# anneouyang/OuterSPACE

Measured on AMD Instinct MI355X. Metric: spgemm_output_nnz_per_s, higher is better.
Workload: dtype f64

## Files before the change

### outerspace_amd/csrc/osp_pipeline.h

```cpp
#pragma once

#define OSP_WITH_RA(ctx_, ...)                                               \
    do {                                                                     \
        if ((ctx_)->rank_atomic) { constexpr bool RA = true; __VA_ARGS__; }  \
        else { constexpr bool RA = false; __VA_ARGS__; }                     \
    } while (0)

template <class T> struct Producer {
    virtual ~Producer() {}
    virtual void produce(uint64_t r0, uint64_t r1, bool whole, uint64_t base, uint64_t count,
                         Part<T> *stage, PhaseTimer &tm, const uint32_t *cells = nullptr, Part<T> *qstage = nullptr,
                         const HubArgs *hub = nullptr, bool compact = false, bool has_long = true, bool desc_only = false, bool walk_all = false) = 0;
};

template <class T> struct MergeIO {
    Part<T> *stage;
    const uint64_t *row_off; uint64_t r0, r1, base;
    int64_t *c_rowptr; uint32_t *c_col; T *c_val;
    const uint64_t *out_in; uint64_t *out_out;
    ChunkTable<T> ct{};
    uint32_t *abort_word = nullptr;
    const RunDesc<T> *runs0 = nullptr; const uint32_t *rowfirst0 = nullptr; const uint32_t *b_colidx = nullptr; const T *b_vals = nullptr;
};
template <class T> struct ShortRuns {
    const RunDesc<T> *runs0 = nullptr; const uint32_t *rowfirst0 = nullptr; const uint32_t *b_colidx = nullptr; const T *b_vals = nullptr;
};

struct TilePlan {
    uint32_t *tile_rows = nullptr;
    uint32_t ntiles = 0;
    uint32_t *long_rows = nullptr;
    uint32_t nlong = 0;
};

static TilePlan plan_tiles(Context *ctx, Scratch &sc, const uint64_t *row_off, uint64_t r0, uint64_t r1, uint64_t base,
                           uint32_t cap, uint32_t max_rows, const uint8_t *force_start, uint64_t total, uint64_t nforce) {
    hipStream_t s = ctx->stream;
    const uint64_t nr = r1 - r0;
    TilePlan pl;
    uint32_t *flag_scan = sc.get<uint32_t>(nr + 1);
    uint32_t *tmp_rows = sc.get<uint32_t>(nr + 1);
    uint64_t *scan_tmp = sc.get<uint64_t>(scan_scratch_entries(std::max<uint64_t>(nr + 1, 16)));
    const uint64_t slot = 8ull * cap;
    CoarseStartFlag csf{row_off, r0, base, slot, force_start};
    device_exclusive_scan<CoarseStartFlag, uint32_t>(csf, nr, flag_scan, (uint32_t *)scan_tmp, s);
    compact_flagged_kernel<CoarseStartFlag><<<grid_for(nr, 256), 256, 0, s>>>(csf, flag_scan, nr, r0, tmp_rows);
    const uint32_t ncb = (uint32_t)std::min<uint64_t>(nr, 2 + nforce + total / slot + nr / 65536);
    const uint32_t *ncb_p = flag_scan + nr;
    uint32_t *cb_cnt = sc.get<uint32_t>((uint64_t)ncb + 1);
    tile_walk_kernel<<<grid_for(ncb, 128), 128, 0, s>>>(tmp_rows, ncb_p, ncb, r1, row_off, cap, max_rows, nullptr, cb_cnt, nullptr);
    device_exclusive_scan<LoadU32, uint32_t>(LoadU32{cb_cnt}, ncb, cb_cnt, (uint32_t *)scan_tmp, s);
    HeavyRowFlag hrf{row_off, r0, cap};
    uint32_t *long_scan = sc.get<uint32_t>(nr + 1);
    uint32_t *long_tmp = sc.get<uint32_t>(scan_scratch_entries(std::max<uint64_t>(nr + 1, 16)));
    device_exclusive_scan<HeavyRowFlag, uint32_t>(hrf, nr, long_scan, long_tmp, s);
    pl.long_rows = sc.get<uint32_t>(nr + 1);
    compact_flagged_kernel<HeavyRowFlag><<<grid_for(nr, 256), 256, 0, s>>>(hrf, long_scan, nr, r0, pl.long_rows);
    { Gather g(s); g.add(&pl.ntiles, (const uint32_t *)cb_cnt + ncb); g.add(&pl.nlong, (const uint32_t *)long_scan + nr); g.wait(); }
    pl.tile_rows = sc.get<uint32_t>((uint64_t)pl.ntiles + 1);
    tile_walk_kernel<<<grid_for(ncb, 128), 128, 0, s>>>(tmp_rows, ncb_p, ncb, r1, row_off, cap, max_rows, cb_cnt, nullptr, pl.tile_rows);
    return pl;
}

struct DirectSrc {
    const uint32_t *rowfirst; const uint64_t *off; const uint32_t *bs; const uint32_t *perm; const uint32_t *b_colidx;
    uint64_t *chunk_off;
    uint64_t direct_max;
    const int64_t *b_rowptr = nullptr;
    uint64_t K = 0, nnz_b = 0;
    Scratch *keep = nullptr;
    mutable HubTables hub{};
    mutable bool hub_refused = false;
    bool gather = false;
    bool expand_rows = false;
    mutable bool chunk_off_ready = true;
    const uint32_t *rows_sorted = nullptr;
    const uint64_t *row_off = nullptr;
    uint64_t rw_cap = 0, nnz = 0;
    void ensure_chunk_off(hipStream_t s) const {
        if (chunk_off_ready) return;
        sym_scatter_offsets_kernel<<<grid_for(nnz, 256), 256, 0, s>>>(perm, off, rows_sorted, row_off, rw_cap, nnz, chunk_off);
        chunk_off_ready = true;
    }
    const void *a_vals = nullptr, *b_vals = nullptr;
    bool av_in_order = false;
    unsigned long long *gstat = nullptr;
};

template <class T> struct PanelPlan {
    Scratch sc;
    TilePlan p0;
    uint32_t max_rows = 0;
    uint64_t *hoff = nullptr, *hscan_tmp = nullptr, *blkbase = nullptr, *hbase = nullptr, *vbase = nullptr, *cellbase = nullptr;
    uint8_t *hbits = nullptr, *hmode = nullptr;
    uint32_t *nstretch = nullptr;
    uint64_t nh = 0, nblocks = 0, nvirt = 0, ncell = 0;
    uint64_t mode_rows[3] = {0, 0, 0}, mode_partials[3] = {0, 0, 0};
    uint32_t *ghist = nullptr, *ghist_tmp = nullptr;
    Part<T> *qstage = nullptr;
    uint64_t *vrow_off = nullptr;
    uint8_t *vfirst = nullptr;
    uint32_t *vcol0 = nullptr, *vcol1 = nullptr;
    uint32_t *cells = nullptr;
    HubArgs hub{};
    GatherArgs<T> ga{};
    uint32_t *vrun_off = nullptr, *vrun_end = nullptr;
    uint32_t *nwritten = nullptr;
    uint64_t *xjobbase = nullptr;
    uint64_t xjobs_bound = 0, xpartials = 0;
    bool expand_ok = false;
    bool may_write = false;
    const DirectSrc *split_from_b = nullptr;
    bool split_beside = false;
    explicit PanelPlan(Context *c) : sc(c) {}
};

__global__ void mode_totals_kernel(const uint32_t *rows, uint32_t nlong, const uint64_t *row_off, const uint8_t *hmode,
                                   const uint8_t *hsmall, unsigned long long *totals) {
    uint64_t part[3] = {0, 0, 0}, cnt[3] = {0, 0, 0}, nsmall = 0;
    for (uint32_t h = blockIdx.x * blockDim.x + threadIdx.x; h < nlong; h += gridDim.x * blockDim.x) {
        const uint64_t U = row_off[rows[h] + 1] - row_off[rows[h]];
        const uint8_t m = hmode[h];
        nsmall += hsmall[h] ? 1ull : 0ull;
#pragma unroll
        for (int mode = 0; mode < 3; mode++) { part[mode] += m == mode ? U : 0ull; cnt[mode] += m == mode ? 1ull : 0ull; }
    }
    for (uint8_t mode = 0; mode < 3; mode++) {
        const uint64_t p = wave_reduce_sum<uint64_t>(part[mode]), c = wave_reduce_sum<uint64_t>(cnt[mode]);
        if (lane_id() == 0 && c) { atomicAdd(&totals[mode], (unsigned long long)c); atomicAdd(&totals[3 + mode], (unsigned long long)p); }
    }
    nsmall = wave_reduce_sum<uint64_t>(nsmall);
    if (lane_id() == 0 && nsmall) atomicAdd(&totals[6], (unsigned long long)nsmall);
}

template <class T>
static void plan_panel(Context *ctx, Result *res, PhaseTimer &tm, PanelPlan<T> &pl, const uint64_t *row_off, uint64_t r0, uint64_t r1,
                       uint64_t base, uint64_t count, int colbits, const DirectSrc *ds) {
    hipStream_t s = ctx->stream;
    Scratch &sc = pl.sc;
    constexpr uint32_t kCap = (uint32_t)TileCap<T>::value;
    pl.max_rows = (uint32_t)std::min<uint64_t>(kTileMaxRows, colbits >= 32 ? 1ull : (1ull << (32 - colbits)));
    pl.p0 = plan_tiles(ctx, sc, row_off, r0, r1, base, kCap, pl.max_rows, nullptr, count, 0);
    res->info.light_tiles += pl.p0.ntiles - pl.p0.nlong;
    if (!pl.p0.nlong) return;
    const uint32_t nlong = pl.p0.nlong;
    pl.hoff = sc.get<uint64_t>((uint64_t)nlong + 1);
    pl.hscan_tmp = sc.get<uint64_t>(scan_scratch_entries(nlong));
    device_exclusive_scan<HeavyLen, uint64_t>(HeavyLen{pl.p0.long_rows, row_off}, nlong, pl.hoff, pl.hscan_tmp, s);
    pl.hbits = sc.get<uint8_t>(nlong);
    pl.hmode = sc.get<uint8_t>(nlong);
    pl.nstretch = sc.get<uint32_t>(nlong);
    uint32_t *nseg = sc.get<uint32_t>(nlong);
    uint64_t *nhist = sc.get<uint64_t>(nlong), *ncellh = sc.get<uint64_t>(nlong);
    const bool want_gather = ds && ds->gather;
    uint64_t *nrund = want_gather ? sc.get<uint64_t>(nlong) : nullptr, *rdbase = want_gather ? sc.get<uint64_t>((uint64_t)nlong + 1) : nullptr;
    uint64_t nrd = 0;
    pl.blkbase = sc.get<uint64_t>((uint64_t)nlong + 1); pl.hbase = sc.get<uint64_t>((uint64_t)nlong + 1);
    pl.vbase = sc.get<uint64_t>((uint64_t)nlong + 1); pl.cellbase = sc.get<uint64_t>((uint64_t)nlong + 1);
    unsigned long long *totals = (unsigned long long *)sc.get<uint64_t>(7);
    uint8_t *hsmall = sc.get<uint8_t>(nlong);
    SmallLimits small_lim{};
    if (want_gather && !(getenv("OSP_PLAN_SMALL") && atoi(getenv("OSP_PLAN_SMALL")) == 0) &&
        !(getenv("OSP_GATHER_OVER") && atoi(getenv("OSP_GATHER_OVER")) == 0)) {
        small_lim.cells = (uint32_t)std::clamp<long>(getenv("OSP_PLAN_SMALL_CELLS") ? atol(getenv("OSP_PLAN_SMALL_CELLS")) : (long)kSmallCells,
                                                     (long)kSmallCellsMin, (long)kSmallCellsMax);
        small_lim.chunks = (uint32_t)std::clamp<long>(getenv("OSP_PLAN_SMALL_CHUNKS") ? atol(getenv("OSP_PLAN_SMALL_CHUNKS")) : (long)kSmallChunks,
                                                      1L, (long)kSmallChunks);
    }
    uint64_t nsmall = 0;
    const uint64_t row_max = getenv("OSP_SPLIT_ROW_MAX") ? strtoull(getenv("OSP_SPLIT_ROW_MAX"), nullptr, 10) : kSplitRowMax;
    const int bits_cap = std::max(colbits - kDenseBits, 1);
    const int hub_b_want = std::min(kSplitMaxBits, bits_cap);
    const bool hub_env = !(getenv("OSP_HUB") && atoi(getenv("OSP_HUB")) == 0);
    int hub_b = 0;
    uint64_t ndcell = 0, tot[6] = {0, 0, 0, 0, 0, 0};
    const int direct_fine = 2;
    const double hub_min_share = getenv("OSP_HUB_MIN_SHARE") ? atof(getenv("OSP_HUB_MIN_SHARE")) : 0.2;
    bool hub_decided = false;
    for (int attempt = 0; attempt < 3; attempt++) {
        const bool hub_possible = ds && ds->b_rowptr && ds->keep && ctx->rank_atomic && hub_env && !ds->hub_refused;
        if (!hub_possible) hub_b = 0;
        split_params_kernel<<<grid_for(nlong, 256), 256, 0, s>>>(pl.p0.long_rows, nlong, row_off, colbits, row_max, bits_cap, ds ? ds->rowfirst : nullptr,
                                                                 ds ? ds->direct_max : 0ull, kCap, pl.hbits, pl.hmode, pl.nstretch, nseg, nhist, ncellh,
                                                                 hub_b, direct_fine, ds ? nrund : nullptr, hsmall, ds ? small_lim : SmallLimits{});
        zero_async(s, {{totals, 7 * sizeof(uint64_t)}});
        mode_totals_kernel<<<std::min(grid_for(nlong, 256), 64u), 256, 0, s>>>(pl.p0.long_rows, nlong, row_off, pl.hmode, hsmall, totals);
        device_exclusive_scan<LoadU32As64, uint64_t>(LoadU32As64{pl.nstretch}, nlong, pl.blkbase, pl.hscan_tmp, s);
        device_exclusive_scan<LoadU32As64, uint64_t>(LoadU32As64{nseg}, nlong, pl.vbase, pl.hscan_tmp, s);
        device_exclusive_scan<LoadU64, uint64_t>(LoadU64{nhist}, nlong, pl.hbase, pl.hscan_tmp, s);
        if (ds) device_exclusive_scan<LoadU64, uint64_t>(LoadU64{ncellh}, nlong, pl.cellbase, pl.hscan_tmp, s);
        if (ds && nrund) device_exclusive_scan<LoadU64, uint64_t>(LoadU64{nrund}, nlong, rdbase, pl.hscan_tmp, s);
        ndcell = 0;
        nrd = 0;
        {
            Gather g(s);
            g.add(&pl.nh, (const uint64_t *)pl.hoff + nlong); g.add(&pl.nblocks, (const uint64_t *)pl.blkbase + nlong);
            g.add(&pl.nvirt, (const uint64_t *)pl.vbase + nlong); g.add(&pl.ncell, (const uint64_t *)pl.hbase + nlong);
            if (ds) g.add(&ndcell, (const uint64_t *)pl.cellbase + nlong);
            if (ds && nrund) g.add(&nrd, (const uint64_t *)rdbase + nlong);
            for (int i = 0; i < 6; i++) g.add(&tot[i], (const uint64_t *)totals + i);
            g.add(&nsmall, (const uint64_t *)totals + 6);
            g.wait();
        }
        if (ds && ndcell >= 0xffffffffull) { ds = nullptr; hub_b = 0; continue; }
        if (hub_possible && !hub_decided && hub_b == 0 && pl.nblocks && (double)tot[3 + kModeStretch] >= hub_min_share * (double)count) {
            hub_decided = true;
            hub_b = hub_b_want;
            continue;
        }
        break;
    }
    for (int m = 0; m < 3; m++) { pl.mode_rows[m] = tot[m]; pl.mode_partials[m] = tot[3 + m]; }
    if (pl.nh >= 0xffffffffull) throw Error(OSP_ERR_CAPACITY, "long rows of one panel exceed 2^32 partial products");
    res->info.heavy_rows += nlong;
    res->info.heavy_partials += pl.nh;
    res->info.direct_rows += pl.mode_rows[kModeDirect];
    res->info.direct_partials += pl.mode_partials[kModeDirect];
    if (pl.ncell >= 0xffffffffull || pl.nblocks >= 0x7fffffffull || pl.nvirt >= 0xffffffffull || ndcell >= 0xffffffffull)
        throw Error(OSP_ERR_CAPACITY, "split histogram too large");
    if (getenv("OSP_VERBOSE"))
        fprintf(stderr, "[osp]   panel rows [%llu,%llu): %u tiles, %u long rows with %llu partial products -> %llu segments; direct: %llu rows, %llu "
                        "partial products, %llu cells\n",
                (unsigned long long)r0, (unsigned long long)r1, pl.p0.ntiles, nlong, (unsigned long long)pl.nh, (unsigned long long)pl.nvirt,
                (unsigned long long)pl.mode_rows[kModeDirect], (unsigned long long)pl.mode_partials[kModeDirect], (unsigned long long)ndcell);
    pl.ghist = sc.get<uint32_t>(pl.ncell + 1);
    pl.ghist_tmp = sc.get<uint32_t>(scan_scratch_entries(pl.ncell + 1));
    pl.vrow_off = sc.get<uint64_t>(pl.nvirt + 1);
    pl.vfirst = sc.get<uint8_t>(pl.nvirt + 1);
    pl.vcol0 = sc.get<uint32_t>(pl.nvirt + 1);
    pl.vcol1 = sc.get<uint32_t>(pl.nvirt + 1);
    if (pl.mode_rows[kModeDirect]) {
        pl.cells = sc.get<uint32_t>(ndcell);
        GatherPlan gp{};
        RunDesc<T> *runs = nullptr;
        static const uint64_t max_runs = getenv("OSP_GATHER_MAX_RUNS") ? strtoull(getenv("OSP_GATHER_MAX_RUNS"), nullptr, 10) : 0xffffffffull;
        if (ds->gather && nrund && nrd < max_runs) {
            runs = sc.get<RunDesc<T>>(std::max<uint64_t>(nrd, 1));
            pl.vrun_off = sc.get<uint32_t>(pl.nvirt + 1);
            pl.vrun_end = sc.get<uint32_t>(pl.nvirt + 1);
            gp.rdbase = rdbase; gp.vrun_off = pl.vrun_off; gp.vrun_end = pl.vrun_end;
            gp.rowruns = sc.get<uint32_t>(nlong);
            pl.nwritten = gp.nwritten = sc.get<uint32_t>(1);
            fill_async(s, {{pl.vrun_off, (pl.nvirt + 1) * sizeof(uint32_t), kNoRuns}, {gp.rowruns, (uint64_t)nlong * sizeof(uint32_t), kNoRuns},
                           {pl.nwritten, sizeof(uint32_t), 0u}});
            gp.over = !(getenv("OSP_GATHER_OVER") && atoi(getenv("OSP_GATHER_OVER")) == 0);
            gp.av_in_order = ds->av_in_order ? 1u : 0u;
            pl.may_write = !gp.over;
            pl.ga.runs = runs; pl.ga.b_colidx = ds->b_colidx; pl.ga.b_vals = (const T *)ds->b_vals;
        }
        if (!(runs && gp.over) || (hub_b && pl.nblocks)) ds->ensure_chunk_off(s);
        gp.mark_skipped = ds->chunk_off_ready ? 1u : 0u;
        const bool plan_small = runs != nullptr && gp.over && nsmall != 0;
        const bool plan_big = !plan_small || nsmall < pl.mode_rows[kModeDirect];
        if (plan_small) gp.small = hsmall;
        if (getenv("OSP_VERBOSE"))
            fprintf(stderr, "[osp]   small planner: %llu of %llu direct rows (at most %u chunks, %u cells)\n", (unsigned long long)(plan_small ? nsmall : 0),
                    (unsigned long long)pl.mode_rows[kModeDirect], small_lim.chunks, small_lim.cells);
        tm.begin(PH_PLAN_K, s);
        if (plan_small)
            direct_plan_small_kernel<T><<<nlong, kWave, direct_plan_small_lds(small_lim.cells), s>>>(
                pl.p0.long_rows, nlong, pl.hbits, nseg, pl.vbase, pl.hoff, colbits, kCap, ds->rowfirst, ds->off, ds->bs, ds->perm, ds->b_colidx,
                pl.vrow_off, pl.vcol0, pl.vcol1, ds->chunk_off, gp, (const T *)ds->a_vals, runs);
        if (!plan_big) {  }
        else if (nlong <= 4u * ctx->cus)
            direct_plan_kernel<T, kDirectCellsBig><<<nlong, kDirectThreads, 0, s>>>(pl.p0.long_rows, nlong, pl.hmode, pl.hbits, nseg, pl.vbase, pl.hoff,
                                                                                 pl.cellbase, row_off, colbits, kCap, ds->rowfirst, ds->off, ds->bs, ds->perm,
                                                                                 ds->b_colidx, pl.vrow_off, pl.vcol0, pl.vcol1, pl.cells, ds->chunk_off, gp,
                                                                                 (const T *)ds->a_vals, runs);
        else
        direct_plan_kernel<T><<<nlong, kDirectThreads, 0, s>>>(pl.p0.long_rows, nlong, pl.hmode, pl.hbits, nseg, pl.vbase, pl.hoff, pl.cellbase, row_off,
                                                              colbits, kCap, ds->rowfirst, ds->off, ds->bs, ds->perm, ds->b_colidx, pl.vrow_off,
                                                              pl.vcol0, pl.vcol1, pl.cells, ds->chunk_off, gp, (const T *)ds->a_vals, runs);
        tm.end(PH_PLAN_K);
        if (gp.rowruns && ds->gstat) gather_stats_kernel<<<std::min(grid_for(nlong, 256), 64u), 256, 0, s>>>(pl.p0.long_rows, nlong, row_off, gp.rowruns, ds->gstat);
#ifdef OSP_PLAN_PROF
        if (getenv("OSP_VERBOSE")) {
            unsigned long long hp[8] = {0}, z[8] = {0};
            OSP_HIP(hipStreamSynchronize(s));
            (void)hipMemcpyFromSymbol(hp, HIP_SYMBOL(osp_plan_prof), sizeof(hp));
            (void)hipMemcpyToSymbol(HIP_SYMBOL(osp_plan_prof), z, sizeof(z));
            double tot = 0;
            for (int k = 0; k < 6; k++) tot += (double)hp[k];
            fprintf(stderr, "[osp]   planner cycles: header %.1f %%, chunk descriptors %.1f %%, histogram pass %.1f %%, grouping %.1f %%, cell pass %.1f %%, "
                            "prefixes + output %.1f %%; %.0f cycles per row, %u rows\n", 100 * hp[0] / tot, 100 * hp[1] / tot, 100 * hp[2] / tot, 100 * hp[3] / tot,
                    100 * hp[4] / tot, 100 * hp[5] / tot, tot / std::max(1u, nlong), nlong);
            (void)hipMemcpyFromSymbol(hp, HIP_SYMBOL(osp_plan_small_prof), sizeof(hp));
            (void)hipMemcpyToSymbol(HIP_SYMBOL(osp_plan_small_prof), z, sizeof(z));
            tot = 0;
            for (int k = 0; k < 5; k++) tot += (double)hp[k];
            if (plan_small && tot > 0)
                fprintf(stderr, "[osp]   small planner cycles: header + chunk descriptors %.1f %%, histogram pass %.1f %%, grouping %.1f %%, counts %.1f %%, "
                                "prefixes + output %.1f %%; %.0f cycles per row, %llu rows\n", 100 * hp[0] / tot, 100 * hp[1] / tot, 100 * hp[2] / tot,
                        100 * hp[3] / tot, 100 * hp[4] / tot, tot / (double)nsmall, (unsigned long long)nsmall);
        }
#endif
        res->info.direct_plan_launches++;
        dbg_sync(s, "plan of the direct rows");
    }
    if (hub_b && pl.nblocks) {
        if (!ds->hub.sx) {
            Scratch &keep = *ds->keep;
            const uint64_t nb = ds->nnz_b;
            Scratch tmp(ctx);
            uint8_t *rowstart = tmp.get<uint8_t>(nb + 4);
            uint32_t *sx = keep.get<uint32_t>(nb + 1), *runstart = keep.get<uint32_t>(nb + 1);
            uint16_t *runblk = keep.get<uint16_t>(nb + 2);
            uint32_t *scan_tmp = tmp.get<uint32_t>(scan_scratch_entries(nb + 1));
            OSP_HIP(hipMemsetAsync(rowstart, 0, nb + 4, s));
            hub_rowstart_kernel<<<grid_for(ds->K, 256), 256, 0, s>>>(ds->b_rowptr, ds->K, rowstart);
            const int sh = colbits - hub_b;
            const HubRunFlag flag{rowstart, ds->b_colidx, sh};
            device_exclusive_scan<HubRunFlag, uint32_t>(flag, nb, sx, scan_tmp, s);
            compact_flagged_kernel<HubRunFlag><<<grid_for(nb, 256), 256, 0, s>>>(flag, sx, nb, 0, runstart);
            hub_runstart_end_kernel<<<1, 1, 0, s>>>(sx + nb, runstart, (uint32_t)nb);
            OSP_HIP(hipMemsetAsync(runblk, 0, (nb + 2) * sizeof(uint16_t), s));
            hub_runblk_kernel<<<std::min(grid_for(nb, 256), 4096u), 256, 0, s>>>(sx + nb, runstart, ds->b_colidx, sh, runblk);
            OSP_HIP(hipStreamSynchronize(s));
            ds->hub.sx = sx; ds->hub.runstart = runstart; ds->hub.runblk = runblk; ds->hub.sh = sh;
        }
        tm.begin(PH_HUB_K, s);
        uint64_t *jobruns = sc.get<uint64_t>(pl.nblocks + 1);
        uint64_t *jobscan_tmp = sc.get<uint64_t>(scan_scratch_entries(pl.nblocks + 1));
        const size_t hub_lds = sizeof(uint32_t) << hub_b;
        hub_plan_kernel<false><<<(unsigned)pl.nblocks, kHubThreads, hub_lds, s>>>(pl.p0.long_rows, nlong, pl.blkbase, pl.hbase, pl.hbits, pl.nstretch, row_off,
                                                                           ds->rowfirst, ds->off, ds->bs, ds->perm, ds->b_colidx, ds->hub, pl.ghist,
                                                                           pl.hoff, jobruns, nullptr, nullptr, nullptr);
        device_exclusive_scan<LoadU32, uint32_t>(LoadU32{pl.ghist}, pl.ncell, pl.ghist, pl.ghist_tmp, s);
        device_exclusive_scan<LoadU64, uint64_t>(LoadU64{jobruns}, pl.nblocks, jobruns, jobscan_tmp, s);
        const uint64_t ncells = d2h(jobruns + pl.nblocks, s);
        if (ncells >= (1ull << 40)) throw Error(OSP_ERR_CAPACITY, "hub rows: too many runs in one panel");
        if (getenv("OSP_VERBOSE"))
            fprintf(stderr, "[osp]   hub rows: %llu rows, %llu products in %llu runs (%.2f records per run), %llu jobs, 2^%d blocks\n",
                    (unsigned long long)pl.mode_rows[kModeStretch], (unsigned long long)pl.mode_partials[kModeStretch], (unsigned long long)ncells,
                    ncells ? (double)pl.mode_partials[kModeStretch] / (double)ncells : 0.0, (unsigned long long)pl.nblocks, hub_b);
        const double min_run = getenv("OSP_HUB_MIN_RUN") ? atof(getenv("OSP_HUB_MIN_RUN")) : 4.0;
        const double run = ncells ? (double)pl.mode_partials[kModeStretch] / (double)ncells : 0.0;
        const bool accept = run >= min_run;
        if (!accept) {
            ds->hub_refused = true;
            tm.end(PH_HUB_K);
        } else {
            uint32_t *hcells = sc.get<uint32_t>(ncells);
            ds->ensure_chunk_off(s);
            hub_plan_kernel<true><<<(unsigned)pl.nblocks, kHubThreads, hub_lds, s>>>(pl.p0.long_rows, nlong, pl.blkbase, pl.hbase, pl.hbits, pl.nstretch, row_off,
                                                                              ds->rowfirst, ds->off, ds->bs, ds->perm, ds->b_colidx, ds->hub, pl.ghist,
                                                                              pl.hoff, nullptr, jobruns, hcells, ds->chunk_off);
            tm.end(PH_HUB_K);
            pl.hub.cells = hcells;
            pl.hub.sx = ds->hub.sx;
            res->info.hub_plan_launches++;
            res->info.hub_cells += ncells;
            res->info.hub_rows += pl.mode_rows[kModeStretch];
            res->info.hub_partials += pl.mode_partials[kModeStretch];
        }
        dbg_sync(s, "plan of the hub rows");
    }
    if (ds && ds->expand_rows) {
        pl.expand_ok = true;
        const bool hubs = pl.hub.cells != nullptr;
        const int from_b_env = getenv("OSP_SPLIT_FROM_B") ? atoi(getenv("OSP_SPLIT_FROM_B")) : 1;
        if (!hubs && pl.nblocks != 0 && from_b_env != 0) pl.split_from_b = ds;
        pl.split_beside = from_b_env != 2;
        const bool stretch_x = !hubs && !pl.split_from_b;
        const uint64_t rows_x = pl.mode_rows[kModeSplitRow] + (stretch_x ? pl.mode_rows[kModeStretch] : 0);
        pl.xpartials = pl.mode_partials[kModeSplitRow] + (stretch_x ? pl.mode_partials[kModeStretch] : 0);
        if (getenv("OSP_VERBOSE") && pl.nblocks && !hubs)
            fprintf(stderr, "[osp]   stretch rows: %llu rows, %llu partial products split %s\n", (unsigned long long)pl.mode_rows[kModeStretch],
                    (unsigned long long)pl.mode_partials[kModeStretch], pl.split_from_b ? (pl.split_beside ? "from B" : "from B, after the join") : "from staged records");
        if (rows_x) {
            pl.xjobbase = sc.get<uint64_t>((uint64_t)nlong + 1);
            device_exclusive_scan<ExpandJobs, uint64_t>(ExpandJobs{pl.p0.long_rows, row_off, pl.hmode, kModeSplitRow, stretch_x ? kModeStretch : kModeSplitRow},
                                                        nlong, pl.xjobbase, pl.hscan_tmp, s);
            pl.xjobs_bound = pl.xpartials / kExpandJob + rows_x;
        }
    }
}

template <class T>
static void split_stretch_from_b(Context *ctx, hipStream_t s, const PanelPlan<T> &pl, const uint64_t *row_off, uint64_t base, int colbits) {
    const DirectSrc *ds = pl.split_from_b;
    const TilePlan &p0 = pl.p0;
    const uint32_t nlong = p0.nlong;
    const uint32_t *perm = ds->av_in_order ? nullptr : ds->perm;
    const RowSrc<float> cols{ds->rowfirst, ds->off, ds->bs, nullptr, nullptr, ds->b_colidx, nullptr};
    const RowSrc<T> src{ds->rowfirst, ds->off, ds->bs, perm, (const T *)ds->a_vals, ds->b_colidx, (const T *)ds->b_vals};
    split_count_kernel<true><<<(unsigned)pl.nblocks, kSplitThreads, 0, s>>>(p0.long_rows, nlong, pl.blkbase, pl.hbase, pl.hbits, pl.nstretch, row_off, base, colbits,
                                                                          nullptr, 0u, pl.ghist, cols);
    device_exclusive_scan<LoadU32, uint32_t>(LoadU32{pl.ghist}, pl.ncell, pl.ghist, pl.ghist_tmp, s);
    OSP_WITH_RA(ctx, split_scatter_kernel<T, RA, true><<<(unsigned)pl.nblocks, kSplitThreads, 0, s>>>(
                         p0.long_rows, nlong, pl.blkbase, pl.hbase, pl.hbits, pl.nstretch, row_off, base, colbits, nullptr, pl.ghist, pl.hoff, pl.qstage, src));
    split_vrows_kernel<<<grid_for(pl.nvirt + 1, 256), 256, 0, s>>>(nlong, pl.vbase, pl.hbase, pl.nstretch, pl.hbits, pl.hmode, colbits, pl.ghist, pl.hoff, pl.nvirt,
                                                                  pl.nh, pl.vrow_off, pl.vfirst, pl.vcol0, pl.vcol1);
    OSP_HIP(hipGetLastError());
}

template <class T>
static void merge_panel(Context *ctx, Result *res, PhaseTimer &tm, const MergeIO<T> &io, int colbits, PanelPlan<T> &pl) {
    hipStream_t s = ctx->stream;
    Scratch &sc = pl.sc;
    constexpr uint32_t kCap = (uint32_t)TileCap<T>::value;
    const uint32_t max_rows = pl.max_rows;
#ifdef OSP_CHECK_DESC
    crumbs_init();
#endif
    const uint64_t r1 = io.r1, base = io.base;
    const TilePlan &p0 = pl.p0;

    MergeLevels<T> lv{};
    lv.stage[0] = io.stage; lv.row_off[0] = io.row_off; lv.base[0] = base; lv.c_rowptr[0] = io.c_rowptr; lv.heavy_nnz[0] = nullptr;
    uint32_t ntot = p0.ntiles;
    TileDesc *desc = nullptr;
    TilePlan p1;
    uint64_t *vbase = pl.vbase;
    int64_t *vptr = nullptr;
    uint64_t *seg_src = nullptr;
    uint32_t *seg_nnz = nullptr;
    Part<T> *qstage = pl.qstage;
    if (p0.nlong) {
        const uint32_t nlong = p0.nlong;
        uint64_t *hoff = pl.hoff, *hscan_tmp = pl.hscan_tmp, *blkbase = pl.blkbase, *hbase = pl.hbase;
        uint8_t *hbits = pl.hbits;
        uint32_t *nstretch = pl.nstretch, *ghist = pl.ghist, *ghist_tmp = pl.ghist_tmp;
        const uint64_t nh = pl.nh, nblocks = pl.nblocks, nvirt = pl.nvirt, ncell = pl.ncell;
        uint64_t *vrow_off = pl.vrow_off;
        uint8_t *vfirst = pl.vfirst;
        if (pl.mode_rows[kModeSplitRow]) {
            tm.begin(PH_SPLIT_K);
            OSP_WITH_RA(ctx, split_row_kernel<T, RA><<<nlong, kSplitRowThreads, 0, s>>>(p0.long_rows, nlong, hbits, pl.hmode, vbase, hoff, io.row_off,
                                                                                     base, colbits, io.stage, qstage, vrow_off));
            tm.end(PH_SPLIT_K);
            res->info.split_launches++;
            res->info.split_partials += pl.mode_partials[kModeSplitRow];
            dbg_sync(s, "split: one-workgroup rows");
        }
        if (pl.split_from_b && !pl.split_beside) split_stretch_from_b<T>(ctx, s, pl, io.row_off, base, colbits);
        if (nblocks && !pl.hub.cells && !pl.split_from_b) {
            split_count_kernel<<<(unsigned)nblocks, kSplitThreads, 0, s>>>(p0.long_rows, nlong, blkbase, hbase, hbits, nstretch, io.row_off,
                                                                         base, colbits, (const char *)io.stage, (uint32_t)sizeof(Part<T>), ghist);
            device_exclusive_scan<LoadU32, uint32_t>(LoadU32{ghist}, ncell, ghist, ghist_tmp, s);
            OSP_WITH_RA(ctx, split_scatter_kernel<T, RA><<<(unsigned)nblocks, kSplitThreads, 0, s>>>(
                                 p0.long_rows, nlong, blkbase, hbase, hbits, nstretch, io.row_off, base, colbits, io.stage, ghist, hoff, qstage));
        }
        dbg_sync(s, "split: stretch rows");
        if (!pl.split_from_b)
            split_vrows_kernel<<<grid_for(nvirt + 1, 256), 256, 0, s>>>(nlong, vbase, hbase, nstretch, hbits, pl.hmode, colbits, ghist, hoff, nvirt, nh,
                                                                       vrow_off, vfirst, pl.vcol0, pl.vcol1);
        OSP_HIP(hipGetLastError());
        dbg_sync(s, "split: segment offsets");
        p1 = plan_tiles(ctx, sc, vrow_off, 0, nvirt, 0, kCap, max_rows, vfirst, nh, nlong);
        dbg_sync(s, "tiles over the segments");
        vptr = (int64_t *)sc.get<uint64_t>(nvirt + 1);
        lv.stage[1] = qstage; lv.row_off[1] = vrow_off; lv.base[1] = 0; lv.c_rowptr[1] = vptr;
        if (p1.nlong) {
            const uint32_t nseg_long = p1.nlong;
            seg_src = sc.get<uint64_t>(nseg_long);
            seg_nnz = sc.get<uint32_t>(nvirt + 1);
            lv.heavy_nnz[1] = seg_nnz;
            if (pl.ga.runs) {
                uint64_t *xsjob = sc.get<uint64_t>((uint64_t)nseg_long + 1);
                uint64_t *xsjob_tmp = sc.get<uint64_t>(scan_scratch_entries((uint64_t)nseg_long + 1));
                device_exclusive_scan<SegExpandJobs, uint64_t>(SegExpandJobs{p1.long_rows, vrow_off, pl.vrun_off}, nseg_long, xsjob, xsjob_tmp, s);
                const uint64_t job_bound = nh / kExpandJob + nseg_long;
                expand_segments_kernel<T><<<(unsigned)std::min<uint64_t>(job_bound, (uint64_t)ctx->cus * 8), kExpandThreads, 0, s>>>(
                    p1.long_rows, nseg_long, xsjob, vrow_off, pl.vrun_off, pl.vrun_end, pl.ga.runs, pl.ga.b_colidx, pl.ga.b_vals, qstage);
            }
            const uint32_t *rest_list = p1.long_rows;
            uint32_t nrest = nseg_long;
            uint32_t *hscan = sc.get<uint32_t>((uint64_t)nseg_long + 1);
            uint64_t *sscan_tmp = sc.get<uint64_t>(scan_scratch_entries(nseg_long));
            {
                const SegDenseFlag df{p1.long_rows, pl.vcol0, pl.vcol1, getenv("OSP_DENSE_SEG") ? atoi(getenv("OSP_DENSE_SEG")) : 1};
                device_exclusive_scan<SegDenseFlag, uint32_t>(df, nseg_long, hscan, (uint32_t *)sscan_tmp, s);
                const uint32_t ndense = d2h(hscan + nseg_long, s);
                if (ndense) {
                    uint32_t *dense_list = sc.get<uint32_t>(ndense), *others = sc.get<uint32_t>(nseg_long - ndense);
                    seg_split_list_kernel<SegDenseFlag><<<grid_for(nseg_long, 256), 256, 0, s>>>(df, hscan, nseg_long, dense_list, others);
                    if (ctx->dense_atomic[sizeof(T) == 8])
                        dense_segment_kernel<T, true><<<grid_for(ndense, kDenseWaves), kDenseWaves * kWave, 0, s>>>(dense_list, ndense, vrow_off, pl.vcol0, pl.vcol1,
                                                                              qstage, seg_nnz);
                    else
                        dense_segment_kernel<T, false><<<grid_for(ndense, kDenseWaves), kDenseWaves * kWave, 0, s>>>(dense_list, ndense, vrow_off, pl.vcol0, pl.vcol1,
                                                                              qstage, seg_nnz);
                    res->info.dense_segments += ndense;
                    rest_list = others;
                    nrest = nseg_long - ndense;
                }
            }
            dbg_sync(s, "over-long segments: dense accumulation");
            const uint32_t big_cap = getenv("OSP_BIGTILE_CAP") ? std::min<uint32_t>((uint32_t)strtoul(getenv("OSP_BIGTILE_CAP"), nullptr, 10), kBigTileCap)
                                                                : (uint32_t)kBigTileCap;
            uint32_t nhuge = 0, nmid = 0;
            uint32_t *huge_list = nullptr, *mid_list = nullptr;
            if (nrest) {
                const SegHugeFlag hf{rest_list, vrow_off, big_cap};
                device_exclusive_scan<SegHugeFlag, uint32_t>(hf, nrest, hscan, (uint32_t *)sscan_tmp, s);
                nhuge = d2h(hscan + nrest, s);
                nmid = nrest - nhuge;
                huge_list = sc.get<uint32_t>(nhuge);
                mid_list = sc.get<uint32_t>(nmid);
                seg_partition_kernel<<<grid_for(nrest, 256), 256, 0, s>>>(hf, hscan, nrest, huge_list, mid_list);
            }
            res->info.sorted_segments += nhuge;
            if (nmid) {
                TileDesc *bdesc = sc.get<TileDesc>(nmid);
                seg_tile_desc_kernel<<<grid_for(nmid, 256), 256, 0, s>>>(mid_list, nmid, vrow_off, pl.vcol0, pl.vcol1, bdesc);
                uint32_t *bticket = sc.get<uint32_t>(1);
                zero_async(s, {{bticket, sizeof(uint32_t)}});
                const uint32_t bgrid = ctx->cus * (uint32_t)merge_wgs_per_cu<T, kBigTileThreads, kBigTileCap>();
                OSP_WITH_RA(ctx, merge_tiles_kernel<T, kBigTileThreads, 32, kBigTileCap, kMergeMaxWgs, RA>
                            <<<std::min<uint32_t>(nmid, bgrid), kBigTileThreads, 0, s>>>(bdesc, nmid, lv, colbits, nullptr, bticket, nullptr, nullptr,
                                                                                         nullptr, nullptr));
            }
            dbg_sync(s, "over-long segments: big in-place tiles");
            if (nhuge) {
                uint64_t *soff = sc.get<uint64_t>((uint64_t)nhuge + 1);
                device_exclusive_scan<HeavyLen, uint64_t>(HeavyLen{huge_list, vrow_off}, nhuge, soff, sscan_tmp, s);
                const uint64_t ns = d2h(soff + nhuge, s);
                res->info.sorted_partials += ns;
                SortedRuns runs(sc, ns);
                heavy_fill_kernel<<<grid_for(ns, 256), 256, 0, s>>>(huge_list, soff, nhuge, vrow_off, 0, colbits, (const char *)qstage,
                                                                    (uint32_t)sizeof(Part<T>), ns, runs.keys[0], runs.poss[0]);
                runs.sort(colbits + bits_for(nhuge));
                T *sorted_val = sc.get<T>(ns);
                heavy_gather_kernel<T><<<grid_for(ns, 256), 256, 0, s>>>(runs.poss[runs.cur], qstage, ns, sorted_val);
                runs.heads();
                heavy_reduce_kernel<T><<<grid_for(ns, 256), 256, 0, s>>>(runs.keys[runs.cur], sorted_val, runs.headscan, runs.head_pos(), ns, huge_list,
                                                                         soff, nhuge, vrow_off, 0, colbits, qstage);
                heavy_rows_kernel<<<grid_for(nhuge, 256), 256, 0, s>>>(huge_list, soff, nhuge, runs.headscan, seg_nnz);
            }
            dbg_sync(s, "over-long segments: global sort");
            heavy_src_inplace_kernel<<<grid_for(nseg_long, 256), 256, 0, s>>>(p1.long_rows, nseg_long, vrow_off, 0, seg_src);
        }
        lv.heavy_nnz[1] = seg_nnz;
        uint32_t *j0 = sc.get<uint32_t>(nlong), *tb = sc.get<uint32_t>((uint64_t)nlong + 1), *extra = sc.get<uint32_t>((uint64_t)nlong + 1);
        chain_rows_kernel<<<grid_for(nlong + 1, 256), 256, 0, s>>>(p0.long_rows, nlong, p0.tile_rows, p0.ntiles, vbase, p1.tile_rows,
                                                                  p1.ntiles, j0, tb, extra);
        device_exclusive_scan<LoadU32, uint32_t>(LoadU32{extra}, nlong, extra, (uint32_t *)hscan_tmp, s);
        ntot = p0.ntiles + (p1.ntiles - nlong);
        desc = sc.get<TileDesc>(ntot);
        tile_desc_kernel<(int)kCap><<<grid_for(p0.ntiles, 256), 256, 0, s>>>(p0.tile_rows, p0.ntiles, r1, io.row_off, base, 0u, j0, extra,
                                                                           nlong, tb, pl.vcol0, pl.vcol1, desc, nullptr, nullptr, io.rowfirst0);
        tile_desc_kernel<(int)kCap><<<grid_for(p1.ntiles, 256), 256, 0, s>>>(p1.tile_rows, p1.ntiles, nvirt, vrow_off, 0, 1u, j0, extra,
                                                                           nlong, tb, pl.vcol0, pl.vcol1, desc, pl.ga.runs ? pl.vrun_off : nullptr,
                                                                           pl.vrun_end);
        dbg_sync(s, "tile chain");
    } else {
        desc = sc.get<TileDesc>(ntot);
        tile_desc_kernel<(int)kCap><<<grid_for(p0.ntiles, 256), 256, 0, s>>>(p0.tile_rows, p0.ntiles, r1, io.row_off, base, 0u, nullptr,
                                                                           nullptr, 0u, nullptr, nullptr, nullptr, desc, nullptr, nullptr, io.rowfirst0);
    }
    uint64_t *tile_status = sc.get<uint64_t>(ntot);
    const uint32_t nshards = 1u;
    uint32_t *ticket = sc.get<uint32_t>((uint64_t)(nshards + 1) * kTicketStride);
    zero_async(s, {{tile_status, (uint64_t)ntot * sizeof(uint64_t)}, {ticket, (uint64_t)(nshards + 1) * kTicketStride * sizeof(uint32_t)}});
    dbg_sync(s, "tile planning, splits, over-long segments");
    tm.begin(PH_MERGE_K);
    if (io.ct.enabled) {
        const uint32_t rw_grid = ctx->cus * (uint32_t)merge_wgs_per_cu<T, kMergeThreads, TileCap<T>::value, kMergeMaxWgs, 64>();
        OSP_WITH_RA(ctx, merge_tiles_kernel<T, kMergeThreads, 64, TileCap<T>::value, kMergeMaxWgs, RA>
                    <<<std::min<uint32_t>(ntot, rw_grid), kMergeThreads, 0, s>>>(desc, ntot, lv, colbits, tile_status, ticket, io.out_in, io.c_col,
                                                                                 io.c_val, io.out_out, io.ct, nshards, io.abort_word));
    } else if (pl.ga.runs || io.runs0) {
        GatherArgs<T> ga = pl.ga;
        ga.runs0 = io.runs0;
        if (io.runs0) { ga.b_colidx = io.b_colidx; ga.b_vals = io.b_vals; }
        const uint32_t merge_grid = ctx->cus * (uint32_t)merge_wgs_per_cu<T, kMergeThreads, TileCap<T>::value>();
        OSP_WITH_RA(ctx, merge_tiles_kernel<T, kMergeThreads, 0, TileCap<T>::value, kMergeMaxWgs, RA, true>
                    <<<std::min<uint32_t>(ntot, merge_grid), kMergeThreads, 0, s>>>(desc, ntot, lv, colbits, tile_status, ticket, io.out_in, io.c_col,
                                                                                    io.c_val, io.out_out, ChunkTable<T>{}, nshards, io.abort_word, ga));
    } else {
        const uint32_t merge_grid = ctx->cus * (uint32_t)merge_wgs_per_cu<T, kMergeThreads, TileCap<T>::value>();
        OSP_WITH_RA(ctx, merge_tiles_kernel<T, kMergeThreads, 0, TileCap<T>::value, kMergeMaxWgs, RA>
                    <<<std::min<uint32_t>(ntot, merge_grid), kMergeThreads, 0, s>>>(desc, ntot, lv, colbits, tile_status, ticket, io.out_in, io.c_col,
                                                                                    io.c_val, io.out_out, ChunkTable<T>{}, nshards, io.abort_word));
    }
    tm.end(PH_MERGE_K);
    dbg_sync(s, "merge tiles");
#ifdef OSP_MERGE_PROF
    if (getenv("OSP_VERBOSE")) {
        std::vector<TileDesc> hd(ntot);
        copy_d2h(hd.data(), desc, (size_t)ntot * sizeof(TileDesc), s);
        uint64_t byp[5] = {0}, ent[5] = {0}, gt = 0, ge = 0, gr = 0, bits[33] = {0};
        for (const TileDesc &t : hd) {
            if (t.n > kCap) continue;
            int rb = 0; while ((1u << rb) < t.nr) rb++;
            const int kb = t.kbits ? (int)t.kbits : colbits + rb;
            const int np = std::min(4, (kb + kDigitBits - 1) / kDigitBits);
            byp[np]++; ent[np] += t.n; bits[std::min(kb, 32)] += 1;
            if (t.rcnt) { gt++; ge += t.n; gr += t.rcnt; }
        }
        fprintf(stderr, "[osp]   tiles by sort passes:");
        for (int k = 0; k < 5; k++) if (byp[k]) fprintf(stderr, " %d passes: %llu tiles, %.0f entries each;", k, (unsigned long long)byp[k], (double)ent[k] / byp[k]);
        fprintf(stderr, " gathered: %llu tiles, %.0f entries and %.1f runs each\n[osp]   tiles by key bits:", (unsigned long long)gt, gt ? (double)ge / gt : 0.0, gt ? (double)gr / gt : 0.0);
        for (int k = 0; k <= 32; k++) if (bits[k]) fprintf(stderr, " %d: %llu;", k, (unsigned long long)bits[k]);
        constexpr int lpt = ((int)kCap + kMergeThreads - 1) / kMergeThreads;
        uint64_t byq[lpt + 1] = {0}, slots = 0, need = 0, run = 0;
        for (const TileDesc &t : hd) {
            if (t.n > kCap) continue;
            const int q = std::max(1, (int)((t.n + kMergeThreads - 1) / kMergeThreads));
            int body = lpt;
            for (int c = kTileRoundClasses; c >= 1; c--) if (q <= tile_class_rounds(lpt, c, kTileRoundClasses)) body = tile_class_rounds(lpt, c, kTileRoundClasses);
            byq[q]++; slots += lpt; need += q; run += body;
        }
        fprintf(stderr, "\n[osp]   tiles by rounds (Q = ceil(n / %d)):", kMergeThreads);
        for (int q = 1; q <= lpt; q++) fprintf(stderr, " Q=%d: %llu;", q, (unsigned long long)byq[q]);
        fprintf(stderr, " slot-rounds needed %.1f %%, run %.1f %% of %d per tile (%d bodies)", slots ? 100.0 * need / slots : 0.0,
                slots ? 100.0 * run / slots : 0.0, lpt, kTileRoundClasses);
        fprintf(stderr, "\n");
    }
    if (getenv("OSP_VERBOSE")) {
        unsigned long long hp[16] = {0}, z[16] = {0};
        OSP_HIP(hipStreamSynchronize(s));
        (void)hipMemcpyFromSymbol(hp, HIP_SYMBOL(osp_merge_prof), sizeof(hp));
        (void)hipMemcpyToSymbol(HIP_SYMBOL(osp_merge_prof), z, sizeof(z));
        static const char *names[12] = {"run table / hash init", "keys + hash count", "publish", "rank", "digit scan", "scatter", "values + heads + scan",
                                        "look-back + ticket", "run sums", "compaction", "output + next tile's request", "gathered: lookup + columns"};
        double tot = 0;
        for (int k = 0; k < 12; k++) tot += (double)hp[k];
        fprintf(stderr, "[osp]   merge kernel, %u tiles, cycles of thread 0 per phase:", ntot);
        for (int k = 0; k < 12; k++) fprintf(stderr, " %s %.1f %%;", names[k], 100.0 * hp[k] / tot);
        fprintf(stderr, " %.0f cycles per tile and workgroup\n", tot / std::max(1u, ntot));
    }
#endif
    res->info.merge_launches++;
    if (p1.nlong) {
        heavy_copy_kernel<T><<<grid_for(p1.nlong, 8), 256, 0, s>>>(p1.long_rows, p1.nlong, seg_src, seg_nnz, vptr, qstage, nullptr, nullptr,
                                                                   io.c_col, io.c_val);
        heavy_copy_rest_kernel<T><<<p1.nlong, 256, 0, s>>>(p1.long_rows, p1.nlong, seg_src, seg_nnz, vptr, qstage, nullptr, nullptr,
                                                           io.c_col, io.c_val);
    }
    chain_finish_kernel<<<grid_for(std::max<uint32_t>(p0.nlong, 1), 256), 256, 0, s>>>(p0.long_rows, p0.nlong, vbase, vptr, io.out_out, r1,
                                                                                       io.c_rowptr);
    dbg_sync(s, "copy of reduced segments, chain finish");
    OSP_HIP(hipGetLastError());
}

struct PanelSink {
    osp_panel_fn fn;
    void *user;
};

constexpr uint64_t kPartialsOnDevice = ~0ull;
template <class T>
static void merge_pipeline(Context *ctx, Result *res, Producer<T> &prod, uint64_t M_all, uint64_t N,
                           const uint64_t *d_row_off,
                           uint64_t P, uint64_t cap_cfg, PhaseTimer &tm, uint64_t r_lo = 0, uint64_t r_hi = ~0ull,
                           uint64_t off_lo = 0, const PanelSink *sink = nullptr, const ChunkTable<T> *ct = nullptr,
                           const DirectSrc *ds = nullptr, const std::vector<uint64_t> *cuts = nullptr, const ShortRuns<T> *sr = nullptr) {
    if (r_hi == ~0ull) r_hi = M_all;
    const uint64_t M = r_hi - r_lo;
    res->info.M = M;
    res->info.row_begin = r_lo;
    res->info.row_end = r_hi;
    hipStream_t s = ctx->stream;
    Scratch sc(ctx);
    const int colbits = std::max(1, bits_for(N));

    const uint64_t E = 4 + sizeof(T);
    uint64_t cap_c;
    uint64_t *ub = sc.get<uint64_t>(M + 1);
    {
        Scratch us(ctx);
        uint64_t *ub_tmp = us.get<uint64_t>(scan_scratch_entries(M + 1));
        if (P != 0) device_exclusive_scan<RowUpperBound, uint64_t>(RowUpperBound{d_row_off + r_lo, N}, M, ub, ub_tmp, s);
        if (P == 0) {
            cap_c = 0;
        } else if (P == kPartialsOnDevice) {
            Gather g(s);
            g.add(&P, d_row_off + M_all);
            g.add(&cap_c, (const uint64_t *)ub + M);
            g.wait();
            res->info.partials = P;
        } else {
            cap_c = d2h(ub + M, s);
        }
    }
    if (!sink) res->rowptr = (int64_t *)ctx->alloc((M + 1) * sizeof(int64_t));
    if (P == 0) {
        res->info.nnz_c = 0;
        if (sink) {
            int64_t *zr = sc.get<int64_t>(M + 1);
            OSP_HIP(hipMemsetAsync(zr, 0, (M + 1) * sizeof(int64_t), s));
            OSP_HIP(hipStreamSynchronize(s));
            res->info.panels = 1;
            const osp_panel_t pd{r_lo, r_hi, 0, zr, nullptr, nullptr, 0, 1, {0, 0}};
            if (sink->fn(&pd, sink->user)) throw Error(OSP_ERR_ARG, "panel callback returned non-zero");
            return;
        }
        OSP_HIP(hipMemsetAsync(res->rowptr, 0, (M + 1) * sizeof(int64_t), s));
        return;
    }
    uint32_t *c_col = nullptr;
    T *c_val = nullptr;
    if (!sink) {
        res->colidx = (uint32_t *)ctx->alloc(std::max<uint64_t>(cap_c, 1) * sizeof(uint32_t));
        res->vals = ctx->alloc(std::max<uint64_t>(cap_c, 1) * sizeof(T));
        c_col = res->colidx;
        c_val = (T *)res->vals;
    }
    size_t free_b = 0, total_b = 0;
    OSP_HIP(hipMemGetInfo(&free_b, &total_b));
    free_b += ctx->pooled_bytes + (ctx->sibling ? ctx->sibling->pooled_bytes : 0);
    uint64_t cap = cap_cfg;
    const double per_record = sink ? 3.7 : (ds && ds->gather) ? 2.5 : 2.6;
    if (cap == 0) cap = std::max<uint64_t>((uint64_t)(free_b * 0.85 / (per_record * E)), 1ull << 20);
    cap = std::min<uint64_t>(cap, 0xfffffff0ull);
    if (getenv("OSP_VERBOSE"))
        fprintf(stderr, "[osp] M=%llu N=%llu P=%llu nnzC<=%llu (%.1f GB) free %.1f GB -> staging capacity %llu partial products (%.1f GB)\n",
                (unsigned long long)M, (unsigned long long)N, (unsigned long long)P, (unsigned long long)cap_c, cap_c * E / 1e9,
                free_b / 1e9, (unsigned long long)cap, cap * E / 1e9);
    std::vector<uint64_t> bounds{r_lo};
    std::vector<uint64_t> boff{off_lo};
    if (P <= cap && !(cuts && !cuts->empty())) {
        bounds.push_back(r_hi);
        boff.push_back(off_lo + P);
    } else {
        constexpr uint32_t kMaxPanels = 4096;
        const uint32_t ncuts = cuts ? (uint32_t)cuts->size() : 0u;
        uint64_t *d_b = sc.get<uint64_t>(2ull * (kMaxPanels + 1) + 2), *d_cuts = sc.get<uint64_t>(std::max<uint32_t>(ncuts, 1));
        if (ncuts) copy_h2d(d_cuts, cuts->data(), ncuts * sizeof(uint64_t), s);
        panel_bounds_kernel<<<1, kWave, 0, s>>>(d_row_off, r_lo, M, cap, d_cuts, ncuts, kMaxPanels, d_b);
        std::vector<uint64_t> hb(2ull * (kMaxPanels + 1) + 2);
        copy_d2h(hb.data(), d_b, hb.size() * sizeof(uint64_t), s);
        const uint64_t np = hb[0], bad = hb[1];
        if (bad != ~0ull)
            throw Error(OSP_ERR_CAPACITY, "output row " + std::to_string(bad) + " has more partial products than the staging capacity of " +
                        std::to_string(cap) + ", or the product needs more than " + std::to_string(kMaxPanels) + " panels");
        for (uint64_t p = 1; p <= np; p++) { bounds.push_back(hb[2 + p]); boff.push_back(hb[2 + (kMaxPanels + 1) + p]); }
        boff[0] = hb[2 + (kMaxPanels + 1)];
    }
    const bool all_rows = r_lo == 0 && r_hi == M_all;
    const uint32_t npanels = (uint32_t)bounds.size() - 1;
    res->info.panels = npanels;
    auto panel_base = [&](uint32_t p) { return (npanels == 1) ? off_lo : boff[p]; };
    auto panel_count = [&](uint32_t p) { return (npanels == 1) ? P : boff[p + 1] - boff[p]; };
    uint64_t max_panel = 0, max_rows_panel = 0;
    for (uint32_t p = 0; p < npanels; p++) {
        max_panel = std::max(max_panel, panel_count(p));
        max_rows_panel = std::max(max_rows_panel, bounds[p + 1] - bounds[p]);
    }
    Part<T> *stage = sc.get<Part<T>>(max_panel);
    uint64_t *out_nnz = sc.get<uint64_t>((uint64_t)npanels + 1);
    uint32_t *abort_word = sc.get<uint32_t>(1);
    zero_async(s, {{out_nnz, sizeof(uint64_t)}, {abort_word, sizeof(uint32_t)}});
    auto check_abort = [&](uint32_t flag) {
        if (flag) throw Error(OSP_ERR_HIP, "the merge made no progress for seconds (a tile's predecessors never published their sizes); "
                                           "with several ticket shards that happens when fewer workgroups than shards ever run side by side");
    };
    const bool overlap = npanels > 1 && !(getenv("OSP_PLAN_OVERLAP") && atoi(getenv("OSP_PLAN_OVERLAP")) == 0);
    if (overlap) ctx->need_aux();
    struct AuxScope {
        Context *c; hipStream_t main;
        explicit AuxScope(Context *ctx_) : c(ctx_), main(ctx_->stream) { c->stream = c->aux; }
        ~AuxScope() {
            if (std::uncaught_exceptions()) (void)hipStreamSynchronize(c->aux);
            c->stream = main;
        }
    };
    typedef std::unique_ptr<PanelPlan<T>> PlanPtr;
    auto plan_one = [&](uint32_t p, bool beside) -> PlanPtr {
        const uint64_t r0 = bounds[p], r1 = bounds[p + 1];
        const uint64_t base = panel_base(p), count = panel_count(p);
        PlanPtr pl(new PanelPlan<T>(ctx));
        if (beside) {
            AuxScope scope(ctx);
            OSP_HIP(hipStreamWaitEvent(ctx->stream, ctx->aux_fork, 0));
            tm.begin(PH_MERGE, ctx->stream);
            plan_panel<T>(ctx, res, tm, *pl, d_row_off, r0, r1, base, count, colbits, ds);
            tm.end(PH_MERGE);
            OSP_HIP(hipEventRecord(ctx->aux_join, ctx->stream));
            res->info.plans_overlapped++;
        } else {
            tm.begin(PH_MERGE);
            plan_panel<T>(ctx, res, tm, *pl, d_row_off, r0, r1, base, count, colbits, ds);
            tm.end(PH_MERGE);
        }
        return pl;
    };
    auto multiply_and_plan_next = [&](uint32_t p, PanelPlan<T> &plan, PlanPtr &nxt) {
        const uint64_t r0 = bounds[p], r1 = bounds[p + 1];
        const uint64_t base = panel_base(p), count = panel_count(p);
        if (plan.p0.nlong) plan.qstage = plan.sc.template get<Part<T>>(plan.nh);
        const bool beside = overlap && p + 1 < npanels;
        if (beside) { OSP_HIP(hipEventRecord(ctx->aux_fork, s)); ctx->fork_window = true; ctx->releases_in_fork_window = 0; }
        struct WindowEnd { Context *c; ~WindowEnd() { c->fork_window = false; } } window_end{ctx};
        tm.begin(PH_MUL);
        bool column_major = count != 0 && !(sr && plan.p0.nlong == 0), desc_only = false;
        if (count && plan.xjobbase && plan.xjobs_bound) {
            tm.begin(PH_EXPAND_K);
            const RowSrc<T> src{ds->rowfirst, ds->off, ds->bs, ds->av_in_order ? nullptr : ds->perm, (const T *)ds->a_vals, ds->b_colidx, (const T *)ds->b_vals};
            expand_rows_kernel<T><<<(unsigned)plan.xjobs_bound, kExpandThreads, 0, s>>>(plan.p0.long_rows, plan.p0.nlong, plan.xjobbase, d_row_off, base, src, stage);
            tm.end(PH_EXPAND_K);
            res->info.expand_launches++;
            res->info.expand_partials += plan.xpartials;
        }
        if (count && plan.split_from_b && plan.split_beside) {
            split_stretch_from_b<T>(ctx, s, plan, d_row_off, base, colbits);
            dbg_sync(s, "split: stretch rows, from B");
        }
        if (count && plan.expand_ok) {
            desc_only = true;
            const uint32_t nw = (plan.nwritten && plan.may_write) ? d2h(plan.nwritten, s) : 0u;
            column_major = plan.hub.cells != nullptr || nw != 0 || (plan.mode_rows[kModeDirect] != 0 && plan.ga.runs == nullptr);
        }
        const bool mostly_hub = plan.hub.cells != nullptr && plan.mode_partials[kModeStretch] * 3 >= count;
        if (column_major && ds) ds->ensure_chunk_off(s);
        if (column_major) prod.produce(r0, r1, npanels == 1 && all_rows, base, count, stage, tm, plan.cells, plan.qstage, plan.hub.cells ? &plan.hub : nullptr,
                                       plan.ga.runs != nullptr && !mostly_hub, plan.p0.nlong != 0, desc_only, mostly_hub);
        tm.end(PH_MUL);
        if (beside) {
            ctx->fork_window = false;
            if (ctx->releases_in_fork_window)
                throw Error(OSP_ERR_HIP, "internal: " + std::to_string(ctx->releases_in_fork_window) + " pooled buffers were released between the fork of the "
                                         "second stream and the next panel's plan (the pool is not stream-aware: see Context::fork_window)");
            nxt = plan_one(p + 1, true);
            OSP_HIP(hipStreamWaitEvent(s, ctx->aux_join, 0));
        }
    };
    if (sink) {
        std::vector<uint64_t> h_ub(npanels + 1);
        for (uint32_t p = 0; p <= npanels; p++) h_ub[p] = d2h(ub + (bounds[p] - r_lo), s);
        uint64_t max_out = 1;
        for (uint32_t p = 0; p < npanels; p++) max_out = std::max(max_out, h_ub[p + 1] - h_ub[p]);
        c_col = sc.get<uint32_t>(max_out);
        c_val = sc.get<T>(max_out);
        int64_t *prow = sc.get<int64_t>(max_rows_panel + 1);
        uint64_t *cells = sc.get<uint64_t>(2);
        uint64_t nnz_total = 0;
        PlanPtr cur, nxt;
        for (uint32_t p = 0; p < npanels; p++) {
            const uint64_t r0 = bounds[p], r1 = bounds[p + 1];
            const uint64_t base = panel_base(p);
            if (!cur) cur = plan_one(p, false);
            PanelPlan<T> &plan = *cur;
            multiply_and_plan_next(p, plan, nxt);
            tm.begin(PH_MERGE);
            OSP_HIP(hipMemsetAsync(cells, 0, 2 * sizeof(uint64_t), s));
            MergeIO<T> io{stage, d_row_off, r0, r1, base, prow - r0, c_col, c_val, cells, cells + 1};
            if (ct) io.ct = *ct;
            if (sr) { io.runs0 = sr->runs0; io.rowfirst0 = sr->rowfirst0; io.b_colidx = sr->b_colidx; io.b_vals = sr->b_vals; }
            io.abort_word = abort_word;
            merge_panel<T>(ctx, res, tm, io, colbits, plan);
            tm.end(PH_MERGE);
            uint64_t nnz_p = 0;
            uint32_t aflag = 0;
            { Gather g(s); g.add(&nnz_p, (const uint64_t *)cells + 1); g.add(&aflag, (const uint32_t *)abort_word); g.wait(); }
            check_abort(aflag);
            nnz_total += nnz_p;
            const osp_panel_t pd{r0, r1, nnz_p, prow, c_col, c_val, p, npanels, {0, 0}};
            ctx->ensure_free(2ull << 30);
            if (sink->fn(&pd, sink->user)) throw Error(OSP_ERR_ARG, "panel callback returned non-zero");
            OSP_HIP(hipStreamSynchronize(s));
            cur = std::move(nxt);
        }
        res->info.nnz_c = nnz_total;
        return;
    }

    PlanPtr cur, nxt;
    for (uint32_t p = 0; p < npanels; p++) {
        const uint64_t r0 = bounds[p], r1 = bounds[p + 1];
        const uint64_t base = panel_base(p);
        if (!cur) cur = plan_one(p, false);
        PanelPlan<T> &plan = *cur;
        multiply_and_plan_next(p, plan, nxt);
        tm.begin(PH_MERGE);
        MergeIO<T> io{stage, d_row_off, r0, r1, base, res->rowptr - r_lo, c_col, c_val, out_nnz + p, out_nnz + p + 1};
        if (ct) io.ct = *ct;
        if (sr) { io.runs0 = sr->runs0; io.rowfirst0 = sr->rowfirst0; io.b_colidx = sr->b_colidx; io.b_vals = sr->b_vals; }
        io.abort_word = abort_word;
        merge_panel<T>(ctx, res, tm, io, colbits, plan);
        tm.end(PH_MERGE);
        cur = std::move(nxt);
    }
    uint64_t nnz_total = 0;
    uint32_t aflag = 0;
    { Gather g(s); g.add(&nnz_total, (const uint64_t *)out_nnz + npanels); g.add(&aflag, (const uint32_t *)abort_word); g.wait(); }
    check_abort(aflag);
    res->info.nnz_c = nnz_total;
    const uint64_t waste = (Context::bucket(std::max<uint64_t>(cap_c, 1) * sizeof(T)) - Context::bucket(std::max<uint64_t>(nnz_total, 1) * sizeof(T))) +
                           (Context::bucket(std::max<uint64_t>(cap_c, 1) * sizeof(uint32_t)) - Context::bucket(std::max<uint64_t>(nnz_total, 1) * sizeof(uint32_t)));
    const uint64_t min_waste = getenv("OSP_COMPACT_MIN_WASTE") ? strtoull(getenv("OSP_COMPACT_MIN_WASTE"), nullptr, 10) : (uint64_t)(total_b / 10);
    res->info.output_slack_bytes = waste;
    if (Context::bucket(std::max<uint64_t>(nnz_total, 1) * sizeof(T)) * 10 < Context::bucket(std::max<uint64_t>(cap_c, 1) * sizeof(T)) * 7 &&
        waste >= min_waste) {
        res->info.output_slack_bytes = 0;
        tm.begin(PH_COMPACT);
        uint32_t *nc = (uint32_t *)ctx->alloc(std::max<uint64_t>(nnz_total, 1) * sizeof(uint32_t));
        T *nv = (T *)ctx->alloc(std::max<uint64_t>(nnz_total, 1) * sizeof(T));
        if (nnz_total) {
            OSP_HIP(hipMemcpyAsync(nc, c_col, nnz_total * sizeof(uint32_t), hipMemcpyDeviceToDevice, s));
            OSP_HIP(hipMemcpyAsync(nv, c_val, nnz_total * sizeof(T), hipMemcpyDeviceToDevice, s));
        }
        ctx->release(res->colidx);
        ctx->release(res->vals);
        res->colidx = nc;
        res->vals = nv;
        tm.end(PH_COMPACT);
    }
}

template <class T> struct OuterProducer : Producer<T> {
    Context *ctx;
    Result *res;
    const int64_t *a_colptr; const uint32_t *a_rowidx; const T *a_vals;
    const int64_t *b_rowptr; const uint32_t *b_colidx; const T *b_vals;
    uint64_t k0, k1; int64_t e0;
    const uint64_t *chunk_off;
    int64_t *a_start; uint32_t *a_cnt; uint64_t *prod; uint64_t *prod_off; uint64_t *scan_tmp;
    bool nothing_staged = false;
    uint32_t *kscan = nullptr, *kscan_tmp = nullptr, *elist = nullptr, *cscan = nullptr, *klist = nullptr;
    uint64_t nnz = 0;
    bool short_gathered = false;
    void produce(uint64_t r0, uint64_t r1, bool whole, uint64_t base, uint64_t count, Part<T> *stage,
                 PhaseTimer &tm, const uint32_t *cells, Part<T> *qstage, const HubArgs *hub = nullptr, bool compact = false, bool has_long = true,
                 bool desc_only = false, bool walk_all = false) override {
        if (nothing_staged) return;
        if (short_gathered && !has_long) return;
        hipStream_t s = ctx->stream;
        const uint64_t nk = k1 - k0;
        const bool ind = (compact || short_gathered) && elist && nnz && !walk_all;
        if (ind) {
            const PanelKeepFlag keep{a_rowidx, chunk_off, e0, (uint32_t)r0, r1, desc_only ? 1u : 0u};
            device_exclusive_scan<PanelKeepFlag, uint32_t>(keep, nnz, kscan, kscan_tmp, s);
            panel_keep_list_kernel<<<grid_for(nnz, 256), 256, 0, s>>>(keep, kscan, nnz, elist);
            const PanelKeepColFlag kcf{a_colptr, e0, k0, kscan};
            device_exclusive_scan<PanelKeepColFlag, uint32_t>(kcf, nk, cscan, kscan_tmp, s);
            panel_keep_columns_kernel<<<grid_for(nk, 256), 256, 0, s>>>(a_colptr, b_rowptr, k0, nk, e0, kscan, cscan, a_start, a_cnt, prod, klist);
        } else {
            panel_columns_kernel<<<grid_for(nk, 256), 256, 0, s>>>(a_colptr, a_rowidx, b_rowptr, k0, nk, (uint32_t)r0, r1,
                                                                   whole ? 1 : 0, a_start, a_cnt, prod);
        }
        device_exclusive_scan<LoadU64, uint64_t>(LoadU64{prod}, nk, prod_off, scan_tmp, s);
        uint64_t nblocks = (count + kMulPerBlock - 1) / kMulPerBlock;
        if (ind) nblocks = std::min<uint64_t>(nblocks, (uint64_t)ctx->cus * 8);
        dbg_sync(s, "panel columns + scan");
        tm.begin(PH_MUL_K);
        if (ind && hub && hub->cells)
            multiply_kernel<T, 2, true><<<(unsigned)nblocks, kMulThreads, 0, s>>>(a_vals, b_colidx, b_vals, b_rowptr, chunk_off, e0,
                                                                                a_start, a_cnt, prod_off, k0, nk, count, base, stage, cells, qstage, *hub, elist, klist);
        else if (ind && cells)
            multiply_kernel<T, 1, true><<<(unsigned)nblocks, kMulThreads, 0, s>>>(a_vals, b_colidx, b_vals, b_rowptr, chunk_off, e0,
                                                                                a_start, a_cnt, prod_off, k0, nk, count, base, stage, cells, qstage, HubArgs{}, elist, klist);
        else if (ind)
            multiply_kernel<T, 0, true><<<(unsigned)nblocks, kMulThreads, 0, s>>>(a_vals, b_colidx, b_vals, b_rowptr, chunk_off, e0,
                                                                                a_start, a_cnt, prod_off, k0, nk, count, base, stage, nullptr, nullptr, HubArgs{}, elist, klist);
        else if (hub && hub->cells)
            multiply_kernel<T, 2><<<(unsigned)nblocks, kMulThreads, 0, s>>>(a_vals, b_colidx, b_vals, b_rowptr, chunk_off, e0,
                                                                          a_start, a_cnt, prod_off, k0, nk, count, base, stage, cells, qstage, *hub);
        else if (cells)
            multiply_kernel<T, 1><<<(unsigned)nblocks, kMulThreads, 0, s>>>(a_vals, b_colidx, b_vals, b_rowptr, chunk_off, e0,
                                                                          a_start, a_cnt, prod_off, k0, nk, count, base, stage, cells, qstage);
        else
            multiply_kernel<T, 0><<<(unsigned)nblocks, kMulThreads, 0, s>>>(a_vals, b_colidx, b_vals, b_rowptr, chunk_off, e0,
                                                                          a_start, a_cnt, prod_off, k0, nk, count, base, stage, nullptr, nullptr);
        tm.end(PH_MUL_K);
        dbg_sync(s, "multiply");
        res->info.multiply_launches++;
    }
};

template <class T> struct PartsProducer : Producer<T> {
    Context *ctx;
    const int64_t *const *d_rowptrs; const uint32_t *const *d_colidxs; const T *const *d_valss;
    int nparts;
    const uint64_t *row_off;
    void produce(uint64_t r0, uint64_t r1, bool, uint64_t base, uint64_t, Part<T> *stage, PhaseTimer &, const uint32_t *, Part<T> *, const HubArgs *, bool, bool, bool, bool) override {
        const uint64_t nr = r1 - r0;
        parts_scatter_kernel<T><<<grid_for(nr * kWave, 256), 256, 0, ctx->stream>>>(d_rowptrs, d_colidxs, d_valss, nparts,
                                                                                    r0, r1, row_off, base, stage);
    }
};

template <class T> struct RecordPartsProducer : Producer<T> {
    Context *ctx;
    const int64_t *const *d_rowptrs; const Part<T> *const *d_recs;
    int nparts;
    const uint64_t *row_off;
    const std::function<void(uint64_t, uint64_t)> *before = nullptr;
    void produce(uint64_t r0, uint64_t r1, bool, uint64_t base, uint64_t, Part<T> *stage, PhaseTimer &, const uint32_t *, Part<T> *, const HubArgs *, bool, bool, bool, bool) override {
        if (before) (*before)(r0, r1);
        const uint64_t nr = r1 - r0;
        parts_scatter_rec_kernel<T><<<grid_for(nr * kWave, 256), 256, 0, ctx->stream>>>(d_rowptrs, d_recs, nparts, r0, r1, row_off, base, stage);
    }
};
```

### outerspace_amd/csrc/osp_prims.h

```cpp
#pragma once
#include <hip/hip_runtime.h>
#include <stdint.h>

#ifndef OSP_RANK_ATOMIC
#define OSP_RANK_ATOMIC 1
#endif

namespace osp {

constexpr int kWave = 64;
constexpr int kScanThreads = 256;
constexpr int kScanItems = 8;
constexpr int kScanTile = kScanThreads * kScanItems;

__device__ __forceinline__ unsigned lane_id() { return threadIdx.x & 63u; }
__device__ __forceinline__ uint64_t lanemask_lt() { return (1ull << lane_id()) - 1ull; }

template <class T>
__device__ __forceinline__ T wave_incl_scan(T v) {
#pragma unroll
    for (int d = 1; d < kWave; d <<= 1) {
        T o = __shfl_up(v, d, kWave);
        if ((int)lane_id() >= d) v += o;
    }
    return v;
}
template <int CTRL, int ROW_MASK>
__device__ __forceinline__ uint32_t dpp_fetch(uint32_t v) {
    return (uint32_t)__builtin_amdgcn_update_dpp(0, (int)v, CTRL, ROW_MASK, 0xf, true);
}
__device__ __forceinline__ uint32_t wave_shr1(uint32_t v) { return dpp_fetch<0x138, 0xf>(v); }
template <>
__device__ __forceinline__ uint32_t wave_incl_scan<uint32_t>(uint32_t v) {
    v += dpp_fetch<0x111, 0xf>(v);
    v += dpp_fetch<0x112, 0xf>(v);
    v += dpp_fetch<0x114, 0xf>(v);
    v += dpp_fetch<0x118, 0xf>(v);
    v += dpp_fetch<0x142, 0xa>(v);
    v += dpp_fetch<0x143, 0xc>(v);
    return v;
}

template <class T>
__device__ __forceinline__ T wave_reduce_sum(T v) {
#pragma unroll
    for (int d = kWave / 2; d > 0; d >>= 1) v += __shfl_down(v, d, kWave);
    return __shfl(v, 0, kWave);
}

__device__ __forceinline__ uint64_t wave_reduce_sum_u62(uint64_t v) {
    const uint32_t a = wave_incl_scan((uint32_t)(v & 0xffffffu));
    const uint32_t b = wave_incl_scan((uint32_t)((v >> 24) & 0xffffffu));
    const uint32_t c = wave_incl_scan((uint32_t)(v >> 48));
    const uint64_t sa = (uint32_t)__builtin_amdgcn_readlane((int)a, 63), sb = (uint32_t)__builtin_amdgcn_readlane((int)b, 63),
                   sc = (uint32_t)__builtin_amdgcn_readlane((int)c, 63);
    return sa + (sb << 24) + (sc << 48);
}

enum { RED_PLUS = 0, RED_MIN = 1, RED_MAX = 2 };
template <int OP, class T>
__device__ __forceinline__ T ordered_identity() {
    return OP == RED_PLUS ? T(0) : OP == RED_MIN ? (T)__builtin_inf() : -(T)__builtin_inf();
}
template <int OP, class T>
__device__ __forceinline__ T ordered_combine(T a, T b) {
#pragma clang fp contract(off)
    return OP == RED_PLUS ? a + b : OP == RED_MIN ? (b < a ? b : a) : (b > a ? b : a);
}
template <int OP, class T>
__device__ __forceinline__ T wave_ordered_reduce(const T *__restrict__ vals, uint64_t m) {
    T p = ordered_identity<OP, T>();
    for (uint64_t i = lane_id(); i < m; i += kWave) p = ordered_combine<OP>(p, vals[i]);
#pragma unroll
    for (int d = kWave / 2; d > 0; d >>= 1) p = ordered_combine<OP>(p, __shfl_down(p, d, kWave));
    return p;
}

template <class T, int NT, bool TAILSYNC = true>
__device__ __forceinline__ T block_excl_scan(T v, T *scratch, T *total) {
    constexpr int NW = NT / kWave;
    const T incl = wave_incl_scan(v);
    const int w = threadIdx.x >> 6;
    if (lane_id() == kWave - 1) scratch[w] = incl;
    __syncthreads();
    T off = 0, tot = 0;
#pragma unroll
    for (int i = 0; i < NW; i++) {
        const T tv = scratch[i];
        if (i < w) off += tv;
        tot += tv;
    }
    *total = tot;
    if (TAILSYNC) __syncthreads();
    return incl - v + off;
}

template <class F, class TOut>
__global__ __launch_bounds__(kScanThreads) void scan_tile_sums_kernel(F f, uint64_t n,
                                                                      TOut *tile_sums) {
    __shared__ TOut scratch[kScanThreads / kWave + 1];
    const uint64_t base = (uint64_t)blockIdx.x * kScanTile;
    TOut s = 0;
#pragma unroll
    for (int i = 0; i < kScanItems; i++) {
        uint64_t idx = base + (uint64_t)i * kScanThreads + threadIdx.x;
        if (idx < n) s += (TOut)f(idx);
    }
    TOut total;
    block_excl_scan<TOut, kScanThreads>(s, scratch, &total);
    if (threadIdx.x == 0) tile_sums[blockIdx.x] = total;
}

template <class TOut>
__global__ __launch_bounds__(kScanThreads) void scan_tile_offsets_kernel(TOut *tile_sums,
                                                                         uint64_t ntiles) {
    __shared__ TOut scratch[kScanThreads / kWave + 1];
    TOut carry = 0;
    for (uint64_t b = 0; b < ntiles; b += kScanThreads) {
        uint64_t i = b + threadIdx.x;
        TOut v = i < ntiles ? tile_sums[i] : (TOut)0;
        TOut total;
        TOut ex = block_excl_scan<TOut, kScanThreads>(v, scratch, &total);
        if (i < ntiles) tile_sums[i] = carry + ex;
        carry += total;
    }
    if (threadIdx.x == 0) tile_sums[ntiles] = carry;
}

template <class F, class TOut>
__global__ __launch_bounds__(kScanThreads) void scan_tiles_kernel(F f, uint64_t n,
                                                                  const TOut *tile_offs,
                                                                  TOut *out) {
    __shared__ TOut scratch[kScanThreads / kWave + 1];
    const uint64_t base = (uint64_t)blockIdx.x * kScanTile;
    TOut v[kScanItems];
    TOut s = 0;
#pragma unroll
    for (int i = 0; i < kScanItems; i++) {
        uint64_t idx = base + (uint64_t)threadIdx.x * kScanItems + i;
        v[i] = idx < n ? (TOut)f(idx) : (TOut)0;
        s += v[i];
    }
    TOut total;
    TOut ex = block_excl_scan<TOut, kScanThreads>(s, scratch, &total) + tile_offs[blockIdx.x];
#pragma unroll
    for (int i = 0; i < kScanItems; i++) {
        uint64_t idx = base + (uint64_t)threadIdx.x * kScanItems + i;
        if (idx < n) out[idx] = ex;
        ex += v[i];
    }
    if (blockIdx.x == gridDim.x - 1 && threadIdx.x == 0) out[n] = tile_offs[gridDim.x];
}

template <class TOut>
__global__ void scan_empty_kernel(TOut *out) { out[0] = 0; }

constexpr uint64_t kScanSmallTiles = 16;
template <class F, class TOut>
__global__ __launch_bounds__(kScanThreads) void scan_small_kernel(F f, uint64_t n, TOut *out) {
    __shared__ TOut scratch[kScanThreads / kWave + 1];
    TOut carry = 0;
    for (uint64_t base = 0; base < n; base += kScanTile) {
        TOut v[kScanItems];
        TOut s = 0;
#pragma unroll
        for (int i = 0; i < kScanItems; i++) {
            const uint64_t idx = base + (uint64_t)threadIdx.x * kScanItems + i;
            v[i] = idx < n ? (TOut)f(idx) : (TOut)0;
            s += v[i];
        }
        TOut total;
        TOut ex = block_excl_scan<TOut, kScanThreads>(s, scratch, &total) + carry;
#pragma unroll
        for (int i = 0; i < kScanItems; i++) {
            const uint64_t idx = base + (uint64_t)threadIdx.x * kScanItems + i;
            if (idx < n) out[idx] = ex;
            ex += v[i];
        }
        carry += total;
    }
    if (threadIdx.x == 0) out[n] = carry;
}

template <class F, class TOut>
inline uint32_t device_exclusive_scan(F f, uint64_t n, TOut *out, TOut *tile_scratch,
                                      hipStream_t stream) {
    if (n == 0) {
        scan_empty_kernel<TOut><<<1, 1, 0, stream>>>(out);
        return 1;
    }
    const uint64_t ntiles = (n + kScanTile - 1) / kScanTile;
    if (ntiles <= kScanSmallTiles) {
        scan_small_kernel<F, TOut><<<1, kScanThreads, 0, stream>>>(f, n, out);
        return 1;
    }
    scan_tile_sums_kernel<F, TOut><<<(unsigned)ntiles, kScanThreads, 0, stream>>>(f, n, tile_scratch);
    scan_tile_offsets_kernel<TOut><<<1, kScanThreads, 0, stream>>>(tile_scratch, ntiles);
    scan_tiles_kernel<F, TOut><<<(unsigned)ntiles, kScanThreads, 0, stream>>>(f, n, tile_scratch, out);
    return 3;
}
inline uint64_t scan_scratch_entries(uint64_t n) { return (n + kScanTile - 1) / kScanTile + 2; }

constexpr int kSortThreads = 256;
constexpr int kSortRounds = 16;
constexpr int kSortTile = kSortThreads * kSortRounds;
constexpr int kRadix = 256;

__device__ __forceinline__ uint64_t wave_match8(unsigned digit, bool valid) {
    uint64_t peers = __ballot(valid);
#pragma unroll
    for (int b = 0; b < 8; b++) {
        const bool bit = (digit >> b) & 1u;
        const uint64_t m = __ballot(bit);
        peers &= bit ? m : ~m;
    }
    return peers;
}

template <class K>
__global__ __launch_bounds__(kSortThreads) void sort_hist_kernel(const K *keys, uint64_t n,
                                                                 int shift, uint32_t *hist,
                                                                 uint32_t nblocks) {
    __shared__ uint32_t h[kRadix];
    h[threadIdx.x] = 0;
    __syncthreads();
    const uint64_t base = (uint64_t)blockIdx.x * kSortTile;
#pragma unroll 4
    for (int r = 0; r < kSortRounds; r++) {
        uint64_t i = base + (uint64_t)r * kSortThreads + threadIdx.x;
        if (i < n) atomicAdd(&h[(unsigned)(keys[i] >> shift) & 255u], 1u);
    }
    __syncthreads();
    hist[(uint64_t)threadIdx.x * nblocks + blockIdx.x] = h[threadIdx.x];
}

template <class K, bool RA>
__global__ __launch_bounds__(kSortThreads) void sort_scatter_kernel(
    const K *keys_in, const uint32_t *vals_in, K *keys_out, uint32_t *vals_out, uint64_t n,
    int shift, const uint32_t *hist_scan, uint32_t nblocks) {
    constexpr int NW = kSortThreads / kWave;
    __shared__ uint32_t base[kRadix];
    __shared__ uint32_t cnt[NW][kRadix];
    base[threadIdx.x] = hist_scan[(uint64_t)threadIdx.x * nblocks + blockIdx.x];
#pragma unroll
    for (int w = 0; w < NW; w++) cnt[w][threadIdx.x] = 0;
    __syncthreads();
    const int w = threadIdx.x >> 6;
    const uint64_t tile = (uint64_t)blockIdx.x * kSortTile;
    for (int r = 0; r < kSortRounds; r++) {
        const uint64_t i = tile + (uint64_t)r * kSortThreads + threadIdx.x;
        const bool valid = i < n;
        K key = 0;
        uint32_t val = 0;
        if (valid) {
            key = keys_in[i];
            val = vals_in[i];
        }
        const unsigned d = (unsigned)(key >> shift) & 255u;
        unsigned rank = 0;
        if constexpr (RA) {
            if (valid) rank = atomicAdd(&cnt[w][d], 1u);
        } else {
            const uint64_t peers = wave_match8(d, valid);
            rank = __popcll(peers & lanemask_lt());
            if (valid && rank == 0) cnt[w][d] = (uint32_t)__popcll(peers);
        }
        __syncthreads();
        if (valid) {
            uint32_t off = base[d] + rank;
#pragma unroll
            for (int ww = 0; ww < NW; ww++)
                if (ww < w) off += cnt[ww][d];
            keys_out[off] = key;
            vals_out[off] = val;
        }
        __syncthreads();
        {
            uint32_t s = 0;
#pragma unroll
            for (int ww = 0; ww < NW; ww++) {
                s += cnt[ww][threadIdx.x];
                cnt[ww][threadIdx.x] = 0;
            }
            base[threadIdx.x] += s;
        }
        __syncthreads();
    }
}

struct LoadU32 {
    const uint32_t *p;
    __device__ uint32_t operator()(uint64_t i) const { return p[i]; }
};

inline uint64_t sort_blocks(uint64_t n) { return (n + kSortTile - 1) / kSortTile; }
inline uint64_t sort_hist_entries(uint64_t n) { return sort_blocks(n) * kRadix + 1; }

struct RadixSorted { int cur; uint32_t launches; };
template <class K>
inline RadixSorted device_radix_sort_pairs(K *keys[2], uint32_t *vals[2], uint64_t n, int nbits,
                                           uint32_t *hist, uint32_t *scan_scratch, hipStream_t stream, bool rank_atomic) {
    int cur = 0;
    uint32_t launches = 0;
    if (n == 0) return {cur, launches};
    const uint32_t nblocks = (uint32_t)sort_blocks(n);
    for (int shift = 0; shift < nbits; shift += 8) {
        sort_hist_kernel<K><<<nblocks, kSortThreads, 0, stream>>>(keys[cur], n, shift, hist, nblocks);
        launches += 2 + device_exclusive_scan<LoadU32, uint32_t>(LoadU32{hist}, (uint64_t)nblocks * kRadix, hist,
                                                                 scan_scratch, stream);
        if (rank_atomic)
            sort_scatter_kernel<K, true><<<nblocks, kSortThreads, 0, stream>>>(keys[cur], vals[cur], keys[cur ^ 1], vals[cur ^ 1], n, shift,
                                                                                hist, nblocks);
        else
            sort_scatter_kernel<K, false><<<nblocks, kSortThreads, 0, stream>>>(keys[cur], vals[cur], keys[cur ^ 1], vals[cur ^ 1], n, shift,
                                                                                 hist, nblocks);
        cur ^= 1;
    }
    return {cur, launches};
}

}
```

Measured before the change: 69.73 billion.

## Replace three-kernel scans with fused single-pass decoupled-lookback scans in planning

Adds a single-pass prefix scan that uses decoupled lookback and handles several independent scans at once. The planning path uses it to fuse the flag scans with compaction, to replace five separate exclusive scans over long rows with one six-way scan, and to scan the histograms in one launch. The goal is fewer kernel launches and fewer passes over memory in the planning phase. In exchange it adds spin-waiting between tiles and an abort path for when lookback stalls, plus extra scratch that must be zeroed.

```diff
diff --git a/outerspace_amd/csrc/osp_onepass_host.h b/outerspace_amd/csrc/osp_onepass_host.h
--- /dev/null
+++ b/outerspace_amd/csrc/osp_onepass_host.h
@@ -0,0 +1,53 @@
+#pragma once
+#include <stdint.h>
+#include <stdlib.h>
+
+#if defined(__HIPCC__) || defined(__CUDACC__)
+#define OSP_HD __host__ __device__ __forceinline__
+#else
+#define OSP_HD inline
+#endif
+
+namespace osp {
+
+constexpr uint64_t kOnepassTile = 2048;
+
+constexpr uint64_t kOnepassAgg = 1ull << 62, kOnepassPrefix = 2ull << 62, kOnepassMask = (1ull << 62) - 1;
+OSP_HD uint64_t onepass_pack(uint64_t flag, uint64_t value) { return flag | (value & kOnepassMask); }
+OSP_HD unsigned onepass_flag(uint64_t w) { return (unsigned)(w >> 62); }
+OSP_HD uint64_t onepass_value(uint64_t w) { return w & kOnepassMask; }
+
+OSP_HD uint64_t onepass_tiles(uint64_t n) { return n ? (n + kOnepassTile - 1) / kOnepassTile : 1; }
+OSP_HD uint64_t onepass_last_tile(uint64_t n) { return n ? (n - 1) / kOnepassTile : 0; }
+OSP_HD bool onepass_tile_leaves(uint64_t t, uint64_t n) { return t != 0 && t * kOnepassTile >= n; }
+OSP_HD uint64_t onepass_scratch_words(uint64_t n_bound, int K) { return 1 + onepass_tiles(n_bound) * (uint64_t)K; }
+
+OSP_HD uint64_t onepass_long_bound(uint64_t rows, uint64_t count, uint64_t cap) {
+    const uint64_t by_len = count / (cap + 1);
+    return rows < by_len ? rows : by_len;
+}
+
+struct OnepassWindow { int p; bool retry; };
+OSP_HD OnepassWindow onepass_window(uint64_t m_prefix, uint64_t m_empty) {
+    OnepassWindow w;
+    w.p = 64;
+    if (m_prefix) w.p = __builtin_ctzll(m_prefix);
+    const uint64_t need = w.p >= 63 ? ~0ull : ((2ull << w.p) - 1ull);
+    w.retry = (m_empty & need) != 0;
+    return w;
+}
+
+struct OnepassCfg {
+    bool on;
+    uint64_t min_tiles;
+};
+inline OnepassCfg onepass_cfg() {
+    OnepassCfg c;
+    const char *e = getenv("OSP_ONEPASS_SCAN"), *m = getenv("OSP_ONEPASS_MIN");
+    c.on = !(e && atoi(e) == 0);
+    c.min_tiles = m ? strtoull(m, nullptr, 10) : 2;
+    if (c.min_tiles < 1) c.min_tiles = 1;
+    return c;
+}
+
+}
diff --git a/outerspace_amd/csrc/osp_pipeline.h b/outerspace_amd/csrc/osp_pipeline.h
--- a/outerspace_amd/csrc/osp_pipeline.h
+++ b/outerspace_amd/csrc/osp_pipeline.h
@@ -34,10 +34,41 @@
 };
 
 static TilePlan plan_tiles(Context *ctx, Scratch &sc, const uint64_t *row_off, uint64_t r0, uint64_t r1, uint64_t base,
-                           uint32_t cap, uint32_t max_rows, const uint8_t *force_start, uint64_t total, uint64_t nforce) {
+                           uint32_t cap, uint32_t max_rows, const uint8_t *force_start, uint64_t total, uint64_t nforce,
+                           uint32_t *abort_word = nullptr, uint64_t extra_words = 0, uint64_t **extra = nullptr) {
     hipStream_t s = ctx->stream;
     const uint64_t nr = r1 - r0;
     TilePlan pl;
+    if (extra) *extra = nullptr;
+    if (onepass_cfg().on) {
+        const uint64_t slot = 8ull * cap;
+        const CoarseStartFlag csf{row_off, r0, base, slot, force_start};
+        const HeavyRowFlag hrf{row_off, r0, cap};
+        const uint32_t ncb = (uint32_t)std::min<uint64_t>(nr, 2 + nforce + total / slot + nr / 65536);
+        const uint64_t w_flags = onepass_scratch_words(nr, 2), w_cb = onepass_scratch_words(ncb, 1);
+        uint64_t *z = sc.get<uint64_t>(w_flags + w_cb + extra_words);
+        zero_async(s, {{z, (w_flags + w_cb + extra_words) * sizeof(uint64_t)}});
+        if (extra) *extra = z + w_flags + w_cb;
+        uint32_t *counts = sc.get<uint32_t>(2);
+        uint32_t *tmp_rows = sc.get<uint32_t>(nr + 1);
+        pl.long_rows = sc.get<uint32_t>(nr + 1);
+        device_onepass_scan(OnepassCompact2<CoarseStartFlag, HeavyRowFlag>{csf, hrf, r0, tmp_rows, pl.long_rows, counts, counts + 1}, nr, nullptr, z,
+                            abort_word, s);
+        uint32_t *cb_cnt = sc.get<uint32_t>((uint64_t)ncb + 1);
+        tile_walk_kernel<<<grid_for(ncb, 128), 128, 0, s>>>(tmp_rows, counts, ncb, r1, row_off, cap, max_rows, nullptr, cb_cnt, nullptr);
+        device_onepass_scan(OnepassPlain<LoadU32, uint32_t>{LoadU32{cb_cnt}, cb_cnt}, ncb, nullptr, z + w_flags, abort_word, s);
+        uint32_t aflag = 0;
+        {
+            Gather g(s);
+            g.add(&pl.ntiles, (const uint32_t *)cb_cnt + ncb); g.add(&pl.nlong, (const uint32_t *)counts + 1);
+            if (abort_word) g.add(&aflag, (const uint32_t *)abort_word);
+            g.wait();
+        }
+        if (aflag) throw Error(OSP_ERR_HIP, "a scan of the tile plan made no progress for seconds (a tile's predecessors never published their sums)");
+        pl.tile_rows = sc.get<uint32_t>((uint64_t)pl.ntiles + 1);
+        tile_walk_kernel<<<grid_for(ncb, 128), 128, 0, s>>>(tmp_rows, counts, ncb, r1, row_off, cap, max_rows, cb_cnt, nullptr, pl.tile_rows);
+        return pl;
+    }
     uint32_t *flag_scan = sc.get<uint32_t>(nr + 1);
     uint32_t *tmp_rows = sc.get<uint32_t>(nr + 1);
     uint64_t *scan_tmp = sc.get<uint64_t>(scan_scratch_entries(std::max<uint64_t>(nr + 1, 16)));
@@ -97,6 +128,7 @@
     uint64_t nh = 0, nblocks = 0, nvirt = 0, ncell = 0;
     uint64_t mode_rows[3] = {0, 0, 0}, mode_partials[3] = {0, 0, 0};
     uint32_t *ghist = nullptr, *ghist_tmp = nullptr;
+    uint64_t *ghist_z = nullptr;
     Part<T> *qstage = nullptr;
     uint64_t *vrow_off = nullptr;
     uint8_t *vfirst = nullptr;
@@ -112,7 +144,57 @@
     bool may_write = false;
     const DirectSrc *split_from_b = nullptr;
     bool split_beside = false;
+    uint32_t *abort_word = nullptr;
     explicit PanelPlan(Context *c) : sc(c) {}
+};
+
+struct PanelScanOp {
+    typedef uint64_t T;
+    static constexpr int K = 6;
+    HeavyLen len;
+    const uint32_t *in32[5];
+    const uint64_t *in64[5];
+    uint64_t *out[6];
+    __device__ void load(uint64_t i, T (&v)[6]) const {
+        v[0] = len(i);
+#pragma unroll
+        for (int k = 0; k < 5; k++) v[k + 1] = in32[k] ? (uint64_t)in32[k][i] : in64[k] ? in64[k][i] : 0ull;
+    }
+    __device__ void store(uint64_t i, const T (&ex)[6], const T (&)[6]) const {
+#pragma unroll
+        for (int k = 0; k < 6; k++)
+            if (out[k]) out[k][i] = ex[k];
+    }
+    __device__ void total(uint64_t n, const T (&tot)[6]) const {
+#pragma unroll
+        for (int k = 0; k < 6; k++)
+            if (out[k]) out[k][n] = tot[k];
+    }
+};
+struct SegPartOp {
+    typedef uint64_t T;
+    static constexpr int K = 3;
+    SegDenseFlag df;
+    SegHugeFlag hf;
+    uint32_t *dense_list, *huge_list, *mid_list;
+    uint64_t *soff, *totals;
+    __device__ void load(uint64_t i, T (&v)[3]) const {
+        const bool dense = df(i) != 0u, huge = !dense && hf(i) != 0u;
+        const uint32_t seg = hf.list[i];
+        v[0] = dense ? 1ull : 0ull;
+        v[1] = huge ? 1ull : 0ull;
+        v[2] = huge ? hf.row_off[seg + 1] - hf.row_off[seg] : 0ull;
+    }
+    __device__ void store(uint64_t i, const T (&ex)[3], const T (&v)[3]) const {
+        const uint32_t seg = hf.list[i];
+        if (v[0]) dense_list[ex[0]] = seg;
+        else if (v[1]) { huge_list[ex[1]] = seg; soff[ex[1]] = ex[2]; }
+        else mid_list[i - ex[0] - ex[1]] = seg;
+    }
+    __device__ void total(uint64_t, const T (&tot)[3]) const {
+        totals[0] = tot[0]; totals[1] = tot[1]; totals[2] = tot[2];
+        soff[tot[1]] = tot[2];
+    }
 };
 
 __global__ void mode_totals_kernel(const uint32_t *rows, uint32_t nlong, const uint64_t *row_off, const uint8_t *hmode,
@@ -140,13 +222,16 @@
     Scratch &sc = pl.sc;
     constexpr uint32_t kCap = (uint32_t)TileCap<T>::value;
     pl.max_rows = (uint32_t)std::min<uint64_t>(kTileMaxRows, colbits >= 32 ? 1ull : (1ull << (32 - colbits)));
-    pl.p0 = plan_tiles(ctx, sc, row_off, r0, r1, base, kCap, pl.max_rows, nullptr, count, 0);
+    const bool onepass = onepass_cfg().on;
+    const uint64_t w_panel = onepass ? onepass_scratch_words(onepass_long_bound(r1 - r0, count, kCap), 6) : 0;
+    uint64_t *zpanel = nullptr;
+    pl.p0 = plan_tiles(ctx, sc, row_off, r0, r1, base, kCap, pl.max_rows, nullptr, count, 0, pl.abort_word, onepass ? w_panel + 7 : 0, &zpanel);
     res->info.light_tiles += pl.p0.ntiles - pl.p0.nlong;
     if (!pl.p0.nlong) return;
     const uint32_t nlong = pl.p0.nlong;
     pl.hoff = sc.get<uint64_t>((uint64_t)nlong + 1);
     pl.hscan_tmp = sc.get<uint64_t>(scan_scratch_entries(nlong));
-    device_exclusive_scan<HeavyLen, uint64_t>(HeavyLen{pl.p0.long_rows, row_off}, nlong, pl.hoff, pl.hscan_tmp, s);
+    if (!onepass) device_exclusive_scan<HeavyLen, uint64_t>(HeavyLen{pl.p0.long_rows, row_off}, nlong, pl.hoff, pl.hscan_tmp, s);
     pl.hbits = sc.get<uint8_t>(nlong);
     pl.hmode = sc.get<uint8_t>(nlong);
     pl.nstretch = sc.get<uint32_t>(nlong);
@@ -157,7 +242,7 @@
     uint64_t nrd = 0;
     pl.blkbase = sc.get<uint64_t>((uint64_t)nlong + 1); pl.hbase = sc.get<uint64_t>((uint64_t)nlong + 1);
     pl.vbase = sc.get<uint64_t>((uint64_t)nlong + 1); pl.cellbase = sc.get<uint64_t>((uint64_t)nlong + 1);
-    unsigned long long *totals = (unsigned long long *)sc.get<uint64_t>(7);
+    unsigned long long *totals = onepass ? (unsigned long long *)(zpanel + w_panel) : (unsigned long long *)sc.get<uint64_t>(7);
     uint8_t *hsmall = sc.get<uint8_t>(nlong);
     SmallLimits small_lim{};
     if (want_gather && !(getenv("OSP_PLAN_SMALL") && atoi(getenv("OSP_PLAN_SMALL")) == 0) &&
@@ -183,6 +268,16 @@
         split_params_kernel<<<grid_for(nlong, 256), 256, 0, s>>>(pl.p0.long_rows, nlong, row_off, colbits, row_max, bits_cap, ds ? ds->rowfirst : nullptr,
                                                                  ds ? ds->direct_max : 0ull, kCap, pl.hbits, pl.hmode, pl.nstretch, nseg, nhist, ncellh,
                                                                  hub_b, direct_fine, ds ? nrund : nullptr, hsmall, ds ? small_lim : SmallLimits{});
+        if (onepass) {
+            if (attempt) zero_async(s, {{zpanel, (w_panel + 7) * sizeof(uint64_t)}});
+            mode_totals_kernel<<<std::min(grid_for(nlong, 256), 64u), 256, 0, s>>>(pl.p0.long_rows, nlong, row_off, pl.hmode, hsmall, totals);
+            PanelScanOp op{};
+            op.len = HeavyLen{pl.p0.long_rows, row_off};
+            op.in32[0] = pl.nstretch; op.in32[1] = nseg; op.in64[2] = nhist; op.in64[3] = ds ? ncellh : nullptr; op.in64[4] = ds ? nrund : nullptr;
+            op.out[0] = pl.hoff; op.out[1] = pl.blkbase; op.out[2] = pl.vbase; op.out[3] = pl.hbase; op.out[4] = ds ? pl.cellbase : nullptr;
+            op.out[5] = (ds && nrund) ? rdbase : nullptr;
+            device_onepass_scan(op, nlong, nullptr, zpanel, pl.abort_word, s);
+        } else {
         zero_async(s, {{totals, 7 * sizeof(uint64_t)}});
         mode_totals_kernel<<<std::min(grid_for(nlong, 256), 64u), 256, 0, s>>>(pl.p0.long_rows, nlong, row_off, pl.hmode, hsmall, totals);
         device_exclusive_scan<LoadU32As64, uint64_t>(LoadU32As64{pl.nstretch}, nlong, pl.blkbase, pl.hscan_tmp, s);
@@ -190,10 +285,13 @@
         device_exclusive_scan<LoadU64, uint64_t>(LoadU64{nhist}, nlong, pl.hbase, pl.hscan_tmp, s);
         if (ds) device_exclusive_scan<LoadU64, uint64_t>(LoadU64{ncellh}, nlong, pl.cellbase, pl.hscan_tmp, s);
         if (ds && nrund) device_exclusive_scan<LoadU64, uint64_t>(LoadU64{nrund}, nlong, rdbase, pl.hscan_tmp, s);
+        }
         ndcell = 0;
         nrd = 0;
+        uint32_t aflag = 0;
         {
             Gather g(s);
+            if (onepass && pl.abort_word) g.add(&aflag, (const uint32_t *)pl.abort_word);
             g.add(&pl.nh, (const uint64_t *)pl.hoff + nlong); g.add(&pl.nblocks, (const uint64_t *)pl.blkbase + nlong);
             g.add(&pl.nvirt, (const uint64_t *)pl.vbase + nlong); g.add(&pl.ncell, (const uint64_t *)pl.hbase + nlong);
             if (ds) g.add(&ndcell, (const uint64_t *)pl.cellbase + nlong);
@@ -202,6 +300,7 @@
             g.add(&nsmall, (const uint64_t *)totals + 6);
             g.wait();
         }
+        if (aflag) throw Error(OSP_ERR_HIP, "the scan over a panel's long rows made no progress for seconds (a tile's predecessors never published their sums)");
         if (ds && ndcell >= 0xffffffffull) { ds = nullptr; hub_b = 0; continue; }
         if (hub_possible && !hub_decided && hub_b == 0 && pl.nblocks && (double)tot[3 + kModeStretch] >= hub_min_share * (double)count) {
             hub_decided = true;
@@ -225,6 +324,9 @@
                 (unsigned long long)pl.mode_rows[kModeDirect], (unsigned long long)pl.mode_partials[kModeDirect], (unsigned long long)ndcell);
     pl.ghist = sc.get<uint32_t>(pl.ncell + 1);
     pl.ghist_tmp = sc.get<uint32_t>(scan_scratch_entries(pl.ncell + 1));
+    const uint64_t w_ghist = (onepass && pl.ncell) ? onepass_scratch_words(pl.ncell, 1) : 0;
+    if (w_ghist) pl.ghist_z = sc.get<uint64_t>(w_ghist);
+    bool ghist_z_clear = w_ghist == 0;
     pl.vrow_off = sc.get<uint64_t>(pl.nvirt + 1);
     pl.vfirst = sc.get<uint8_t>(pl.nvirt + 1);
     pl.vcol0 = sc.get<uint32_t>(pl.nvirt + 1);
@@ -242,7 +344,8 @@
             gp.rowruns = sc.get<uint32_t>(nlong);
             pl.nwritten = gp.nwritten = sc.get<uint32_t>(1);
             fill_async(s, {{pl.vrun_off, (pl.nvirt + 1) * sizeof(uint32_t), kNoRuns}, {gp.rowruns, (uint64_t)nlong * sizeof(uint32_t), kNoRuns},
-                           {pl.nwritten, sizeof(uint32_t), 0u}});
+                           {pl.nwritten, sizeof(uint32_t), 0u}, {pl.ghist_z, w_ghist * sizeof(uint64_t), 0u}});
+            ghist_z_clear = true;
             gp.over = !(getenv("OSP_GATHER_OVER") && atoi(getenv("OSP_GATHER_OVER")) == 0);
             gp.av_in_order = ds->av_in_order ? 1u : 0u;
             pl.may_write = !gp.over;
@@ -297,6 +400,7 @@
         res->info.direct_plan_launches++;
         dbg_sync(s, "plan of the direct rows");
     }
+    if (!ghist_z_clear) zero_async(s, {{pl.ghist_z, w_ghist * sizeof(uint64_t)}});
     if (hub_b && pl.nblocks) {
         if (!ds->hub.sx) {
             Scratch &keep = *ds->keep;
@@ -386,7 +490,8 @@
     const RowSrc<T> src{ds->rowfirst, ds->off, ds->bs, perm, (const T *)ds->a_vals, ds->b_colidx, (const T *)ds->b_vals};
     split_count_kernel<true><<<(unsigned)pl.nblocks, kSplitThreads, 0, s>>>(p0.long_rows, nlong, pl.blkbase, pl.hbase, pl.hbits, pl.nstretch, row_off, base, colbits,
                                                                           nullptr, 0u, pl.ghist, cols);
-    device_exclusive_scan<LoadU32, uint32_t>(LoadU32{pl.ghist}, pl.ncell, pl.ghist, pl.ghist_tmp, s);
+    if (pl.ghist_z) device_onepass_scan(OnepassPlain<LoadU32, uint32_t>{LoadU32{pl.ghist}, pl.ghist}, pl.ncell, nullptr, pl.ghist_z, pl.abort_word, s);
+    else device_exclusive_scan<LoadU32, uint32_t>(LoadU32{pl.ghist}, pl.ncell, pl.ghist, pl.ghist_tmp, s);
     OSP_WITH_RA(ctx, split_scatter_kernel<T, RA, true><<<(unsigned)pl.nblocks, kSplitThreads, 0, s>>>(
                          p0.long_rows, nlong, pl.blkbase, pl.hbase, pl.hbits, pl.nstretch, row_off, base, colbits, nullptr, pl.ghist, pl.hoff, pl.qstage, src));
     split_vrows_kernel<<<grid_for(pl.nvirt + 1, 256), 256, 0, s>>>(nlong, pl.vbase, pl.hbase, pl.nstretch, pl.hbits, pl.hmode, colbits, pl.ghist, pl.hoff, pl.nvirt,
@@ -437,7 +542,8 @@
         if (nblocks && !pl.hub.cells && !pl.split_from_b) {
             split_count_kernel<<<(unsigned)nblocks, kSplitThreads, 0, s>>>(p0.long_rows, nlong, blkbase, hbase, hbits, nstretch, io.row_off,
                                                                          base, colbits, (const char *)io.stage, (uint32_t)sizeof(Part<T>), ghist);
-            device_exclusive_scan<LoadU32, uint32_t>(LoadU32{ghist}, ncell, ghist, ghist_tmp, s);
+            if (pl.ghist_z) device_onepass_scan(OnepassPlain<LoadU32, uint32_t>{LoadU32{ghist}, ghist}, ncell, nullptr, pl.ghist_z, pl.abort_word, s);
+            else device_exclusive_scan<LoadU32, uint32_t>(LoadU32{ghist}, ncell, ghist, ghist_tmp, s);
             OSP_WITH_RA(ctx, split_scatter_kernel<T, RA><<<(unsigned)nblocks, kSplitThreads, 0, s>>>(
                                  p0.long_rows, nlong, blkbase, hbase, hbits, nstretch, io.row_off, base, colbits, io.stage, ghist, hoff, qstage));
         }
@@ -447,7 +553,11 @@
                                                                        vrow_off, vfirst, pl.vcol0, pl.vcol1);
         OSP_HIP(hipGetLastError());
         dbg_sync(s, "split: segment offsets");
-        p1 = plan_tiles(ctx, sc, vrow_off, 0, nvirt, 0, kCap, max_rows, vfirst, nh, nlong);
+        const bool onepass = onepass_cfg().on;
+        const uint64_t nseg_bound = onepass_long_bound(nvirt, nh, kCap);
+        const uint64_t w_x = onepass_scratch_words(nseg_bound, 1), w_part = onepass_scratch_words(nseg_bound, 3), w_chain = onepass_scratch_words(nlong, 1);
+        uint64_t *zmerge = nullptr;
+        p1 = plan_tiles(ctx, sc, vrow_off, 0, nvirt, 0, kCap, max_rows, vfirst, nh, nlong, io.abort_word, onepass ? w_x + w_part + w_chain + 1 : 0, &zmerge);
         dbg_sync(s, "tiles over the segments");
         vptr = (int64_t *)sc.get<uint64_t>(nvirt + 1);
         lv.stage[1] = qstage; lv.row_off[1] = vrow_off; lv.base[1] = 0; lv.c_rowptr[1] = vptr;
@@ -459,6 +569,10 @@
             if (pl.ga.runs) {
                 uint64_t *xsjob = sc.get<uint64_t>((uint64_t)nseg_long + 1);
                 uint64_t *xsjob_tmp = sc.get<uint64_t>(scan_scratch_entries((uint64_t)nseg_long + 1));
+                if (onepass)
+                    device_onepass_scan(OnepassPlain<SegExpandJobs, uint64_t>{SegExpandJobs{p1.long_rows, vrow_off, pl.vrun_off}, xsjob}, nseg_long, nullptr,
+                                        zmerge, io.abort_word, s);
+                else
                 device_exclusive_scan<SegExpandJobs, uint64_t>(SegExpandJobs{p1.long_rows, vrow_off, pl.vrun_off}, nseg_long, xsjob, xsjob_tmp, s);
                 const uint64_t job_bound = nh / kExpandJob + nseg_long;
                 expand_segments_kernel<T><<<(unsigned)std::min<uint64_t>(job_bound, (uint64_t)ctx->cus * 8), kExpandThreads, 0, s>>>(
@@ -468,6 +582,42 @@
             uint32_t nrest = nseg_long;
             uint32_t *hscan = sc.get<uint32_t>((uint64_t)nseg_long + 1);
             uint64_t *sscan_tmp = sc.get<uint64_t>(scan_scratch_entries(nseg_long));
+            const uint32_t big_cap = getenv("OSP_BIGTILE_CAP") ? std::min<uint32_t>((uint32_t)strtoul(getenv("OSP_BIGTILE_CAP"), nullptr, 10), kBigTileCap)
+                                                                : (uint32_t)kBigTileCap;
+            uint32_t nhuge = 0, nmid = 0;
+            uint32_t *huge_list = nullptr, *mid_list = nullptr;
+            uint64_t *soff = nullptr, ns = 0;
+            if (onepass) {
+                const SegDenseFlag df{p1.long_rows, pl.vcol0, pl.vcol1, getenv("OSP_DENSE_SEG") ? atoi(getenv("OSP_DENSE_SEG")) : 1};
+                const SegHugeFlag hf{p1.long_rows, vrow_off, big_cap};
+                uint32_t *dense_list = sc.get<uint32_t>(nseg_long);
+                huge_list = sc.get<uint32_t>(nseg_long);
+                mid_list = sc.get<uint32_t>(nseg_long);
+                soff = sc.get<uint64_t>((uint64_t)nseg_long + 1);
+                uint64_t *part_totals = sc.get<uint64_t>(3);
+                device_onepass_scan(SegPartOp{df, hf, dense_list, huge_list, mid_list, soff, part_totals}, nseg_long, nullptr, zmerge + w_x, io.abort_word, s);
+                uint64_t ndense64 = 0, nhuge64 = 0;
+                uint32_t aflag = 0;
+                {
+                    Gather g(s);
+                    g.add(&ndense64, (const uint64_t *)part_totals); g.add(&nhuge64, (const uint64_t *)part_totals + 1); g.add(&ns, (const uint64_t *)part_totals + 2);
+                    if (io.abort_word) g.add(&aflag, (const uint32_t *)io.abort_word);
+                    g.wait();
+                }
+                if (aflag) throw Error(OSP_ERR_HIP, "a scan over a panel's over-long segments made no progress for seconds (a tile's predecessors never published their sums)");
+                const uint32_t ndense = (uint32_t)ndense64;
+                nhuge = (uint32_t)nhuge64;
+                nmid = nseg_long - ndense - nhuge;
+                if (ndense) {
+                    if (ctx->dense_atomic[sizeof(T) == 8])
+                        dense_segment_kernel<T, true><<<grid_for(ndense, kDenseWaves), kDenseWaves * kWave, 0, s>>>(dense_list, ndense, vrow_off, pl.vcol0, pl.vcol1,
+                                                                              qstage, seg_nnz);
+                    else
+                        dense_segment_kernel<T, false><<<grid_for(ndense, kDenseWaves), kDenseWaves * kWave, 0, s>>>(dense_list, ndense, vrow_off, pl.vcol0, pl.vcol1,
+                                                                              qstage, seg_nnz);
+                    res->info.dense_segments += ndense;
+                }
+            } else {
             {
                 const SegDenseFlag df{p1.long_rows, pl.vcol0, pl.vcol1, getenv("OSP_DENSE_SEG") ? atoi(getenv("OSP_DENSE_SEG")) : 1};
                 device_exclusive_scan<SegDenseFlag, uint32_t>(df, nseg_long, hscan, (uint32_t *)sscan_tmp, s);
@@ -487,10 +637,6 @@
                 }
             }
             dbg_sync(s, "over-long segments: dense accumulation");
-            const uint32_t big_cap = getenv("OSP_BIGTILE_CAP") ? std::min<uint32_t>((uint32_t)strtoul(getenv("OSP_BIGTILE_CAP"), nullptr, 10), kBigTileCap)
-                                                                : (uint32_t)kBigTileCap;
-            uint32_t nhuge = 0, nmid = 0;
-            uint32_t *huge_list = nullptr, *mid_list = nullptr;
             if (nrest) {
                 const SegHugeFlag hf{rest_list, vrow_off, big_cap};
                 device_exclusive_scan<SegHugeFlag, uint32_t>(hf, nrest, hscan, (uint32_t *)sscan_tmp, s);
@@ -500,12 +646,13 @@
                 mid_list = sc.get<uint32_t>(nmid);
                 seg_partition_kernel<<<grid_for(nrest, 256), 256, 0, s>>>(hf, hscan, nrest, huge_list, mid_list);
             }
+            }
             res->info.sorted_segments += nhuge;
             if (nmid) {
                 TileDesc *bdesc = sc.get<TileDesc>(nmid);
                 seg_tile_desc_kernel<<<grid_for(nmid, 256), 256, 0, s>>>(mid_list, nmid, vrow_off, pl.vcol0, pl.vcol1, bdesc);
-                uint32_t *bticket = sc.get<uint32_t>(1);
-                zero_async(s, {{bticket, sizeof(uint32_t)}});
+                uint32_t *bticket = onepass ? (uint32_t *)(zmerge + w_x + w_part + w_chain) : sc.get<uint32_t>(1);
+                if (!onepass) zero_async(s, {{bticket, sizeof(uint32_t)}});
                 const uint32_t bgrid = ctx->cus * (uint32_t)merge_wgs_per_cu<T, kBigTileThreads, kBigTileCap>();
                 OSP_WITH_RA(ctx, merge_tiles_kernel<T, kBigTileThreads, 32, kBigTileCap, kMergeMaxWgs, RA>
                             <<<std::min<uint32_t>(nmid, bgrid), kBigTileThreads, 0, s>>>(bdesc, nmid, lv, colbits, nullptr, bticket, nullptr, nullptr,
@@ -513,9 +660,11 @@
             }
             dbg_sync(s, "over-long segments: big in-place tiles");
             if (nhuge) {
-                uint64_t *soff = sc.get<uint64_t>((uint64_t)nhuge + 1);
-                device_exclusive_scan<HeavyLen, uint64_t>(HeavyLen{huge_list, vrow_off}, nhuge, soff, sscan_tmp, s);
-                const uint64_t ns = d2h(soff + nhuge, s);
+                if (!onepass) {
+                    soff = sc.get<uint64_t>((uint64_t)nhuge + 1);
+                    device_exclusive_scan<HeavyLen, uint64_t>(HeavyLen{huge_list, vrow_off}, nhuge, soff, sscan_tmp, s);
+                    ns = d2h(soff + nhuge, s);
+                }
                 res->info.sorted_partials += ns;
                 SortedRuns runs(sc, ns);
                 heavy_fill_kernel<<<grid_for(ns, 256), 256, 0, s>>>(huge_list, soff, nhuge, vrow_off, 0, colbits, (const char *)qstage,
@@ -535,7 +684,8 @@
         uint32_t *j0 = sc.get<uint32_t>(nlong), *tb = sc.get<uint32_t>((uint64_t)nlong + 1), *extra = sc.get<uint32_t>((uint64_t)nlong + 1);
         chain_rows_kernel<<<grid_for(nlong + 1, 256), 256, 0, s>>>(p0.long_rows, nlong, p0.tile_rows, p0.ntiles, vbase, p1.tile_rows,
                                                                   p1.ntiles, j0, tb, extra);
-        device_exclusive_scan<LoadU32, uint32_t>(LoadU32{extra}, nlong, extra, (uint32_t *)hscan_tmp, s);
+        if (onepass) device_onepass_scan(OnepassPlain<LoadU32, uint32_t>{LoadU32{extra}, extra}, nlong, nullptr, zmerge + w_x + w_part, io.abort_word, s);
+        else device_exclusive_scan<LoadU32, uint32_t>(LoadU32{extra}, nlong, extra, (uint32_t *)hscan_tmp, s);
         ntot = p0.ntiles + (p1.ntiles - nlong);
         desc = sc.get<TileDesc>(ntot);
         tile_desc_kernel<(int)kCap><<<grid_for(p0.ntiles, 256), 256, 0, s>>>(p0.tile_rows, p0.ntiles, r1, io.row_off, base, 0u, j0, extra,
@@ -762,6 +912,7 @@
         const uint64_t r0 = bounds[p], r1 = bounds[p + 1];
         const uint64_t base = panel_base(p), count = panel_count(p);
         PlanPtr pl(new PanelPlan<T>(ctx));
+        pl->abort_word = abort_word;
         if (beside) {
             AuxScope scope(ctx);
             OSP_HIP(hipStreamWaitEvent(ctx->stream, ctx->aux_fork, 0));
diff --git a/outerspace_amd/csrc/osp_prims.h b/outerspace_amd/csrc/osp_prims.h
--- a/outerspace_amd/csrc/osp_prims.h
+++ b/outerspace_amd/csrc/osp_prims.h
@@ -1,6 +1,7 @@
 #pragma once
 #include <hip/hip_runtime.h>
 #include <stdint.h>
+#include "osp_onepass_host.h"
 
 #ifndef OSP_RANK_ATOMIC
 #define OSP_RANK_ATOMIC 1
@@ -200,6 +201,218 @@
     return 3;
 }
 inline uint64_t scan_scratch_entries(uint64_t n) { return (n + kScanTile - 1) / kScanTile + 2; }
+
+static_assert(kOnepassTile == (uint64_t)kScanTile, "osp_onepass_host.h and osp_prims.h disagree about the scan tile");
+constexpr uint32_t kOnepassSpinLimit = 1u << 22;
+struct OnepassCtl {
+    uint64_t n;
+    const uint32_t *n_dev;
+    uint64_t *scratch;
+    uint32_t *abort_word;
+    uint32_t single;
+};
+
+template <int K>
+__device__ __forceinline__ void onepass_lookback(uint64_t *status, uint32_t t, const uint64_t (&total)[K], uint64_t (&excl)[K], uint32_t *abort_word) {
+    const unsigned lane = lane_id();
+    if (lane == 0) {
+#pragma unroll
+        for (int k = 0; k < K; k++)
+            __hip_atomic_store(&status[(uint64_t)t * K + k], onepass_pack(t == 0 ? kOnepassPrefix : kOnepassAgg, total[k]), __ATOMIC_RELAXED,
+                               __HIP_MEMORY_SCOPE_AGENT);
+    }
+    bool done[K];
+#pragma unroll
+    for (int k = 0; k < K; k++) { excl[k] = 0; done[k] = false; }
+    int64_t b = (int64_t)t - 1;
+    uint32_t spins = 0;
+    while (b >= 0) {
+        const int64_t idx = b - (int64_t)lane;
+        uint64_t sv[K];
+        int p[K];
+        bool retry = false;
+#pragma unroll
+        for (int k = 0; k < K; k++) {
+            sv[k] = kOnepassPrefix;
+            if (idx >= 0) sv[k] = __hip_atomic_load(&status[(uint64_t)idx * K + k], __ATOMIC_RELAXED, __HIP_MEMORY_SCOPE_AGENT);
+            const OnepassWindow w = onepass_window(__ballot(onepass_flag(sv[k]) == 2u), __ballot(onepass_flag(sv[k]) == 0u));
+            p[k] = w.p;
+            retry = retry || (!done[k] && w.retry);
+        }
+        if (retry) {
+            __builtin_amdgcn_s_sleep(1);
+            if ((++spins & 255u) == 0) {
+                const bool give_up = spins >= kOnepassSpinLimit;
+                if (give_up && lane == 0 && abort_word) atomicExch(abort_word, 1u);
+                if (give_up || (abort_word && __hip_atomic_load(abort_word, __ATOMIC_RELAXED, __HIP_MEMORY_SCOPE_AGENT) != 0u)) break;
+            }
+            continue;
+        }
+        bool all = true;
+#pragma unroll
+        for (int k = 0; k < K; k++) {
+            if (!done[k]) {
+                excl[k] += wave_reduce_sum_u62((int)lane <= p[k] ? onepass_value(sv[k]) : 0ull);
+                if (p[k] < 64) done[k] = true;
+            }
+            all = all && done[k];
+        }
+        if (all) break;
+        b -= kWave;
+    }
+    if (lane == 0 && t != 0) {
+#pragma unroll
+        for (int k = 0; k < K; k++)
+            __hip_atomic_store(&status[(uint64_t)t * K + k], onepass_pack(kOnepassPrefix, excl[k] + total[k]), __ATOMIC_RELAXED, __HIP_MEMORY_SCOPE_AGENT);
+    }
+}
+
+template <class Op>
+__global__ __launch_bounds__(kScanThreads) void onepass_scan_kernel(const Op op, const OnepassCtl c) {
+    typedef typename Op::T T;
+    constexpr int K = Op::K;
+    constexpr int NW = kScanThreads / kWave;
+    __shared__ T wsum[K][NW];
+    __shared__ uint64_t pre_s[K];
+    __shared__ uint32_t tile_s;
+    uint64_t n = c.n;
+    if (c.n_dev) n = min(n, (uint64_t)*c.n_dev);
+    if (!c.single) {
+        if (threadIdx.x == 0) tile_s = atomicAdd((uint32_t *)c.scratch, 1u);
+        __syncthreads();
+    }
+    uint32_t t = c.single ? 0u : tile_s;
+    if (onepass_tile_leaves(t, n)) return;
+    const unsigned w = threadIdx.x >> 6;
+    T carry[K];
+#pragma unroll
+    for (int k = 0; k < K; k++) carry[k] = 0;
+    for (;;) {
+        const uint64_t base = (uint64_t)t * kScanTile + (uint64_t)threadIdx.x * kScanItems;
+        T v[kScanItems][K], ex[K];
+#pragma unroll
+        for (int k = 0; k < K; k++) ex[k] = 0;
+#pragma unroll
+        for (int i = 0; i < kScanItems; i++) {
+#pragma unroll
+            for (int k = 0; k < K; k++) v[i][k] = 0;
+            if (base + i < n) op.load(base + i, v[i]);
+#pragma unroll
+            for (int k = 0; k < K; k++) ex[k] += v[i][k];
+        }
+        T tot[K];
+#pragma unroll
+        for (int k = 0; k < K; k++) {
+            const T incl = wave_incl_scan(ex[k]);
+            if (lane_id() == kWave - 1) wsum[k][w] = incl;
+            ex[k] = incl - ex[k];
+        }
+        __syncthreads();
+#pragma unroll
+        for (int k = 0; k < K; k++) {
+            T off = 0, s = 0;
+#pragma unroll
+            for (int i = 0; i < NW; i++) {
+                const T tv = wsum[k][i];
+                if (i < (int)w) off += tv;
+                s += tv;
+            }
+            ex[k] += off;
+            tot[k] = s;
+        }
+        if (c.single) {
+#pragma unroll
+            for (int k = 0; k < K; k++) ex[k] += carry[k];
+        } else {
+            if (threadIdx.x < kWave) {
+                uint64_t tot64[K], excl[K];
+#pragma unroll
+                for (int k = 0; k < K; k++) tot64[k] = (uint64_t)tot[k];
+                onepass_lookback<K>(c.scratch + 1, t, tot64, excl, c.abort_word);
+                if (threadIdx.x == 0) {
+#pragma unroll
+                    for (int k = 0; k < K; k++) pre_s[k] = excl[k];
+                }
+            }
+            __syncthreads();
+#pragma unroll
+            for (int k = 0; k < K; k++) { carry[k] = (T)pre_s[k]; ex[k] += carry[k]; }
+        }
+#pragma unroll
+        for (int i = 0; i < kScanItems; i++) {
+            if (base + i < n) op.store(base + i, ex, v[i]);
+#pragma unroll
+            for (int k = 0; k < K; k++) ex[k] += v[i][k];
+        }
+#pragma unroll
+        for (int k = 0; k < K; k++) carry[k] += tot[k];
+        if ((uint64_t)t == onepass_last_tile(n)) {
+            if (threadIdx.x == 0) op.total(n, carry);
+            break;
+        }
+        if (!c.single) break;
+        t++;
+        __syncthreads();
+    }
+}
+
+inline bool onepass_single(uint64_t n_bound) { return onepass_tiles(n_bound) < onepass_cfg().min_tiles || onepass_tiles(n_bound) == 1; }
+template <class Op>
+inline uint32_t device_onepass_scan(const Op &op, uint64_t n_bound, const uint32_t *n_dev, uint64_t *scratch, uint32_t *abort_word, hipStream_t stream) {
+    const bool single = onepass_single(n_bound) || !scratch;
+    const OnepassCtl c{n_bound, n_dev, scratch, abort_word, single ? 1u : 0u};
+    onepass_scan_kernel<Op><<<single ? 1u : (unsigned)onepass_tiles(n_bound), kScanThreads, 0, stream>>>(op, c);
+    return 1;
+}
+
+template <class F, class TOut>
+struct OnepassPlain {
+    typedef TOut T;
+    static constexpr int K = 1;
+    F f;
+    TOut *out;
+    __device__ void load(uint64_t i, T (&v)[1]) const { v[0] = (TOut)f(i); }
+    __device__ void store(uint64_t i, const T (&ex)[1], const T (&)[1]) const { out[i] = ex[0]; }
+    __device__ void total(uint64_t n, const T (&tot)[1]) const { out[n] = tot[0]; }
+};
+template <class F0, class F1>
+struct OnepassCompact2 {
+    typedef uint32_t T;
+    static constexpr int K = 2;
+    F0 f0;
+    F1 f1;
+    uint64_t r0;
+    uint32_t *list0, *list1;
+    uint32_t *count0, *count1;
+    __device__ void load(uint64_t i, T (&v)[2]) const { v[0] = f0(i) ? 1u : 0u; v[1] = f1(i) ? 1u : 0u; }
+    __device__ void store(uint64_t i, const T (&ex)[2], const T (&v)[2]) const {
+        if (v[0]) list0[ex[0]] = (uint32_t)(r0 + i);
+        if (v[1]) list1[ex[1]] = (uint32_t)(r0 + i);
+    }
+    __device__ void total(uint64_t, const T (&tot)[2]) const { *count0 = tot[0]; *count1 = tot[1]; }
+};
+template <int KK>
+struct OnepassArrays {
+    typedef uint64_t T;
+    static constexpr int K = KK;
+    const uint32_t *in32[KK];
+    const uint64_t *in64[KK];
+    uint64_t *out[KK];
+    __device__ void load(uint64_t i, T (&v)[KK]) const {
+#pragma unroll
+        for (int k = 0; k < KK; k++) v[k] = in32[k] ? (uint64_t)in32[k][i] : in64[k] ? in64[k][i] : 0ull;
+    }
+    __device__ void store(uint64_t i, const T (&ex)[KK], const T (&)[KK]) const {
+#pragma unroll
+        for (int k = 0; k < KK; k++)
+            if (out[k]) out[k][i] = ex[k];
+    }
+    __device__ void total(uint64_t n, const T (&tot)[KK]) const {
+#pragma unroll
+        for (int k = 0; k < KK; k++)
+            if (out[k]) out[k][n] = tot[k];
+    }
+};
 
 constexpr int kSortThreads = 256;
 constexpr int kSortRounds = 16;
```

Result: no change. 70.18 billion, median of 6 (+0.6%).
